# TurakhiaLab/TWILIGHT

Hardware: AMD Instinct MI355X
Metric: DP band cells/s, TALCO-XDrop progressive profile-profile alignment (bit-exact vs reference CPU path) (higher is better)
Workload: dtype f32

## Files before the change

### __graft_entry__.py

```python
from __future__ import annotations

import os
import subprocess
import sys

ROOT = os.path.dirname(os.path.abspath(__file__))
CSRC = os.path.join(ROOT, "twilight_amd", "csrc")
LIB = os.path.join(ROOT, "twilight_amd", "libtwl_align.so")
HIPCC = os.environ.get("HIPCC", "/opt/rocm/bin/hipcc")
KERNEL_SOURCES = ("twl_align.hip", "twl_knobs.inc.hip", "twl_launch.inc.hip", "twl_policy.inc.hip", "twl_run.inc.hip", "twl_comm.inc.hip", "talco_exit.hip.h", "talco_kernel.hip.h", "talco_nuc.hip.h", "talco_lds.hip.h", "talco_div.hip.h", "talco_team.hip.h", "talco_mt.hip.h", "talco_global.hip.h", "twl_level_plan.inc.hip", "twl_store.inc.hip", "twl_level.inc.hip", "level_kernels.hip.h", "restore_kernels.hip.h", "twl_place.inc.hip", "place_kernels.hip.h",
                  "twl_merge.inc.hip", "twl_merge_plan.inc.hip", "merge_kernels.hip.h", "twl_path_source.inc.hip", "twl_place_plan.inc.hip",
                  "twl_subtree.inc.hip", "twl_subtree_plan.inc.hip", "subtree_kernels.hip.h",
                  "twl_guide.inc.hip", "twl_guide_plan.inc.hip", "guide_kernels.hip.h",
                  "twl_guide_set.inc.hip", "twl_guide_set_plan.inc.hip", "guide_stage_kernels.hip.h",
                  "twl_strand.inc.hip", "twl_strand_plan.inc.hip", "strand_kernels.hip.h",
                  "twl_retree.inc.hip", "twl_retree_plan.inc.hip", "retree_kernels.hip.h",
                  "twl_retree_set.inc.hip", "twl_retree_set_plan.inc.hip", "retree_stage_kernels.hip.h",
                  "twl_backbone.inc.hip", "twl_backbone_plan.inc.hip", "backbone_kernels.hip.h",
                  "twl_keep.inc.hip", "twl_keep_plan.inc.hip", "keep_kernels.hip.h")
HIP_FLAGS = ["--offload-arch=gfx950", "-O2", "-ffp-contract=off", "-fno-slp-vectorize", "-fPIC", "-shared", "-std=c++17"]
HOST_FLAGS = ["-O2", "-std=c++17", "-fopenmp", "-ffp-contract=off", "-Wall"]

_STATE: dict = {}


def _digest(files, extra=()) -> str:
    import hashlib
    h = hashlib.sha256()
    for f in files:
        h.update(os.path.basename(f).encode() + b"\0")
        h.update(open(f, "rb").read())
    for e in extra:
        h.update(str(e).encode() + b"\0")
    return h.hexdigest()[:16]


def _stamped(target, stamp) -> bool:
    if not os.path.exists(target):
        return False
    return (b"TWLSTAMP:" + stamp.encode() + b";") in open(target, "rb").read()


def source_hash() -> str:
    import hashlib
    h = hashlib.sha256()
    for f in KERNEL_SOURCES:
        h.update(open(os.path.join(CSRC, f), "rb").read())
    return h.hexdigest()[:12]


def build_state() -> dict:
    return dict(_STATE)


def build() -> None:
    srcs = [os.path.join(CSRC, f) for f in KERNEL_SOURCES] + \
           [os.path.join(ROOT, "include", h) for h in ("twl_align.h", "twl_level.h", "twl_place.h", "twl_merge.h", "twl_subtree.h", "twl_guide.h", "twl_strand.h", "twl_retree.h", "twl_retree_set.h", "twl_backbone.h", "twl_keep.h")]
    flags = HIP_FLAGS + (["-DTWL_DEV"] if os.environ.get("TWL_DEV_BUILD") else [])
    stamp = _digest(srcs, flags)
    if _stamped(LIB, stamp):
        _STATE["libtwl_align.so"] = "current"
    else:
        subprocess.check_call([HIPCC] + flags + [f'-DTWL_SOURCE_HASH="{source_hash()}"', f'-DTWL_BUILD_STAMP="{stamp}"', "-o", LIB,
                               os.path.join(CSRC, "twl_align.hip")], cwd=CSRC)
        _STATE["libtwl_align.so"] = "built"
    host = os.path.join(CSRC, "host")
    lib_srcs = [os.path.join(host, f) for f in ("phylo.cpp", "seqdb_io.cpp", "helpers.cpp", "progressive.cpp", "driver.cpp", "align_gpu.cpp", "align_resident.cpp", "align_owned.cpp", "capi.cpp", "place.cpp", "merge.cpp", "partition.cpp", "subtrees.cpp", "guide.cpp", "retree.cpp", "place_tree.cpp", "strand.cpp")]
    hdrs = [os.path.join(host, h) for h in ("twl_host.hpp", "align_gpu.hpp", "level_policy.hpp", "exchange_plan.hpp", "guide_upgma.hpp", "guide_stage.hpp", "strand_orient.hpp")] + \
           [os.path.join(ROOT, "include", h) for h in ("twl_msa.h", "twl_align.h", "twl_level.h", "twl_place.h", "twl_merge.h", "twl_subtree.h", "twl_guide.h", "twl_strand.h", "twl_retree.h", "twl_retree_set.h", "twl_backbone.h", "twl_keep.h")] + \
           [os.path.join(CSRC, "twl_retree_plan.inc.hip")]
    hostlib = os.path.join(ROOT, "twilight_amd", "libtwl_host.so")
    hstamp = _digest(lib_srcs + hdrs, HOST_FLAGS + [stamp])
    if _stamped(hostlib, hstamp):
        _STATE["libtwl_host.so"] = "current"
    else:
        subprocess.check_call(["g++"] + HOST_FLAGS + [f'-DTWL_BUILD_STAMP="{hstamp}"', "-fPIC", "-shared", "-o", hostlib] + lib_srcs +
                              [LIB, "-Wl,-rpath,$ORIGIN", "-lz"], cwd=host)
        _STATE["libtwl_host.so"] = "built"
    exe = os.path.join(ROOT, "twilight_amd", "twilight-mi355x")
    exe_flags = HOST_FLAGS + ["-DTWL_PLACE", "-DTWL_MERGE", "-DTWL_SUBTREE", "-DTWL_GUIDE"]
    estamp = _digest([os.path.join(host, "main.cpp")] + hdrs, exe_flags + [hstamp])
    if _stamped(exe, estamp):
        _STATE["twilight-mi355x"] = "current"
    else:
        subprocess.check_call(["g++"] + exe_flags + [f'-DTWL_BUILD_STAMP="{estamp}"', "-o", exe, os.path.join(host, "main.cpp"),
                               hostlib, LIB, "-Wl,-rpath,$ORIGIN", "-lz"], cwd=host)
        _STATE["twilight-mi355x"] = "built"
    subprocess.check_call(["make", "-C", os.path.join(ROOT, "oracle"), "all"], stdout=subprocess.DEVNULL)
    sys.path.insert(0, ROOT)
    import twilight_amd

    twilight_amd.load_library()
    check_not_stale()
# ... 43 lines not shown
```

### include/twl_align.h

```cpp
#ifndef TWL_ALIGN_H
#define TWL_ALIGN_H

#include <stdint.h>

#ifdef __cplusplus
extern "C" {
#endif

#define TWL_MAX_MATRIX 21
#define TWL_MAX_MARKER 1024

enum twl_status {
    TWL_OK = 0,
    TWL_ERR_NOT_INITIALIZED = -1,
    TWL_ERR_BAD_ARGUMENT = -2,
    TWL_ERR_HIP = -3,
    TWL_ERR_UNSUPPORTED = -4
};

typedef struct twl_params {
    int32_t P;
    float   matrix[TWL_MAX_MATRIX * TWL_MAX_MATRIX];
    float   gap_open;
    float   gap_extend;
    float   gap_boundary;
    float   gap_char;
    int32_t xdrop;
    int32_t flen;
    int32_t marker;
} twl_params;

typedef struct twl_stats {
    uint64_t band_cells;
    uint64_t nominal_cells;
    double   kernel_ms;
    double   pack_ms;
    double   total_ms;
    int32_t  n_launches;
    int32_t  n_relaunched;
    int32_t  window;
    int32_t  grid;
    int32_t  matrix_mode;
    int32_t  speculative;
    int32_t  mt_tiles_predicted;
    int32_t  mt_tiles_inline;
    int32_t  mt_scouts_failed;
    int32_t  reserved;
    char     kernel[160];
} twl_stats;

int  twl_init(const int *device_ids, int n_devices);
void twl_shutdown(void);
const char *twl_last_error(void);
const char *twl_version(void);

int twl_align_batch(const twl_params *p, int32_t n_pairs, int32_t seq_len,
                    const float *freq, const float *gap_open, const float *gap_extend,
                    const int32_t *len, const int32_t *num,
                    int8_t *aln_out, int32_t *aln_len_out, int16_t *err_out);

int twl_align_batch_device(int device, void *stream, const twl_params *p, int32_t n_pairs, int32_t seq_len,
                           const float *d_freq, const float *d_gap_open, const float *d_gap_extend,
                           const int32_t *d_len, const int32_t *d_num,
                           int8_t *d_aln_out, int32_t *d_aln_len_out, int16_t *d_err_out);

void *twl_host_alloc(uint64_t bytes);
void  twl_host_free(void *p);

int twl_copy_to_device(int device, void *dst_dev, const void *src, uint64_t bytes);
int twl_copy_from_device(int device, void *dst, const void *src_dev, uint64_t bytes);
int twl_copy_rows_from_device(int device, void *dst, uint64_t dst_pitch, const void *src_dev, uint64_t src_pitch, uint64_t width, uint64_t rows);

int twl_get_stats(int device, twl_stats *out);

int twl_get_pair_cells(int device, uint64_t *cells_out, int32_t n);

int twl_column_scores(const twl_params *p, int32_t seq_len, const float *freq, const int32_t *len, const int32_t *num, float *out);

int twl_dp_column_scores(const twl_params *p, int32_t seq_len, const float *freq, const float *gap_open, const float *gap_extend,
                         const int32_t *len, const int32_t *num, float *out);

#define TWL_MT_REC_WORDS 12
typedef struct twl_mt_dims {
    int32_t n_run, slots, sp_pitch, segcap;
    int32_t n_scout, n_tile, rounds;
    int32_t lead2, marg, anchors;
    int32_t thr, small_tiles, marker;
    int32_t reserved[3];
} twl_mt_dims;
int twl_mt_tables(int device, twl_mt_dims *dims, int32_t *order, int32_t *anchor, int32_t *spath, int32_t *chain, int32_t *rec, int8_t *seg, int32_t *front);

#define TWL_COMM_ID_BYTES 128
int twl_comm_unique_id(void *id128);
int twl_comm_init(int device, int rank, int world, const void *id128);
int twl_comm_all_gather(int device, const void *d_send, void *d_recv, int64_t bytes_per_rank);
int twl_comm_all_gather_host(int device, const void *send, void *recv, int64_t bytes_per_rank);
int twl_comm_destroy(int device);

enum twl_knob { TWL_KNOB_MT_PERTURB = 1, TWL_KNOB_MT_MAX_PAIRS = 2, TWL_KNOB_MT_MIN_MARKER = 3, TWL_KNOB_MT_LEAD = 4, TWL_KNOB_MT_MARGIN = 5,
                TWL_KNOB_MT_ROUNDS = 6, TWL_KNOB_MT_THR_JOBS = 7, TWL_KNOB_FAIL_ROW_ALLOCS = 8,
                TWL_KNOB_PROT_MODE = 9, TWL_KNOB_ASSUME_ONEHOT_QUERY = 10, TWL_KNOB_MT_TAIL_PCT = 11, TWL_KNOB_MT_WIDE = 12, TWL_KNOB_NO_SPEC = 13, TWL_KNOB_SCOUT_XDROP_PCT = 14, TWL_KNOB_THR_SMALL = 15, TWL_KNOB_FORCE_GLOBAL = 16, TWL_KNOB_LEAF_STEP = 17, TWL_KNOB_POISON_TB = 18, TWL_KNOB_MT_ANCHOR = 19, TWL_KNOB_MT_LEAD2 = 20, TWL_KNOB_PROT_CORRIDOR = 21, TWL_KNOB_TAIL_OVERLAP = 22 };
int twl_set_knob(int key, int value);
int twl_plan_describe(const twl_params *p, int32_t n_pairs, const int32_t *len, int32_t num_cu, int32_t qry_onehot, int32_t wide_streak, char *out, int32_t cap);

#ifdef __cplusplus
}
#endif
#endif
```

### include/twl_level.h

```cpp
#ifndef TWL_LEVEL_H
#define TWL_LEVEL_H

#include "twl_align.h"

#ifdef __cplusplus
extern "C" {
#endif

typedef struct twl_store twl_store;

typedef struct twl_side {
    int32_t n_members;
    int32_t member_off;
    int32_t len;
    int32_t num;
    float   weight;
    int32_t cache_id;
    int32_t store_id;
    int32_t reserved;
} twl_side;

int  twl_store_create(int device, char type, int32_t n_seqs, const char *const *seqs, const int32_t *lens, twl_store **out);
void twl_store_destroy(twl_store *s);
int  twl_store_read_rows(twl_store *s, char *const *rows_out, int32_t *lens_out);
int  twl_store_read_rows_of(twl_store *s, int32_t n_ids, const int32_t *ids, char *out, int32_t *lens_out);
int  twl_store_write_rows(twl_store *s, int32_t n_ids, const int32_t *ids, const char *in, const int32_t *lens);
int  twl_store_write_cache(twl_store *s, int32_t id, const float *data, int32_t len);
int  twl_store_rows_to_block(twl_store *s, int32_t n_ids, const int32_t *ids, void *dev_block, int32_t *lens_out);
int  twl_store_rows_from_block(twl_store *s, int32_t n_ids, const int32_t *ids, const int32_t *lens, const void *dev_block);
int  twl_store_exchange_buffers(twl_store *s, int64_t send_bytes, int64_t recv_bytes, void **send_dev, void **recv_dev);
int  twl_store_read_cache(twl_store *s, int32_t id, float *out, int32_t *len_out);
int  twl_store_drop_cache(twl_store *s, int32_t id);

int twl_level_prepare(twl_store *s, const twl_params *p, float gappy_threshold, int32_t n_pairs, const twl_side *sides,
                      const int32_t *members, const float *member_weight, int32_t seq_len, int32_t *len_out, uint8_t *colinfo_out);

int twl_level_read_colinfo(twl_store *s, int32_t pair, int32_t side, uint8_t *out);
int twl_level_read_colinfo_many(twl_store *s, int32_t n_sel, const int32_t *pairs, uint8_t *out);

int twl_level_align(twl_store *s, const twl_params *p, const uint8_t *run_mask, int8_t *aln_out, int32_t *aln_len_out, int16_t *err_out);
int twl_level_align_mixed(twl_store *s, const twl_params *p, const uint8_t *run_mask, const uint8_t *zero_gap, int8_t *aln_out, int32_t *aln_len_out, int16_t *err_out);

int twl_level_read_path(twl_store *s, int32_t pair, int8_t *out, int32_t len);
int twl_level_read_paths(twl_store *s, int32_t n_sel, const int32_t *pairs, const int32_t *lens, int8_t *out, int32_t out_stride);

int twl_level_restore(twl_store *s, const twl_params *p, int32_t n_sel, const int32_t *pairs, int32_t out_stride, int32_t *final_len_out);
int twl_level_exchange_buffers(twl_store *s, int64_t send_bytes, int64_t recv_bytes, void **send_dev, void **recv_dev);
int twl_level_paths_to_block(twl_store *s, int32_t n_sel, const int32_t *pairs, const int32_t *lens, const uint8_t *where, void *blk_dev, const int64_t *blk_off);
int twl_level_paths_from_block(twl_store *s, int32_t n_sel, const int32_t *pairs, const int32_t *lens, const void *blk_dev, const int64_t *blk_off);
int twl_level_write_final(twl_store *s, int32_t pair, const int8_t *path, int32_t len);
int twl_level_read_final(twl_store *s, int32_t pair, int8_t *out, int32_t len);

int twl_level_commit(twl_store *s, const int8_t *paths, const int32_t *path_len, int32_t path_stride);

int twl_level_commit_from_dp(twl_store *s, const int8_t *paths, const int32_t *path_len, int32_t path_stride, const uint8_t *from_dp);

int twl_level_read_columns(twl_store *s, int32_t pair, int32_t side, float *out, int32_t max_cols);

int twl_level_timing(twl_store *s, double *prepare_ms, double *commit_ms);

#ifdef __cplusplus
}
#endif
#endif
```

### twilight_amd/api.py

```python
from __future__ import annotations

import ctypes as C
import os

import numpy as np

_HERE = os.path.dirname(os.path.abspath(__file__))
LIB_PATH = os.environ.get("TWL_LIB") or os.path.join(_HERE, "libtwl_align.so")
TWL_MAX_MATRIX = 21

_lib = None


class TwlError(RuntimeError):
    pass


class TwlParams(C.Structure):
    _fields_ = [("P", C.c_int32), ("matrix", C.c_float * (TWL_MAX_MATRIX * TWL_MAX_MATRIX)), ("gap_open", C.c_float),
                ("gap_extend", C.c_float), ("gap_boundary", C.c_float), ("gap_char", C.c_float), ("xdrop", C.c_int32),
                ("flen", C.c_int32), ("marker", C.c_int32)]


class TwlStats(C.Structure):
# ... 45 lines not shown
        lib.twl_set_knob.restype = C.c_int
        lib.twl_mt_tables.restype = C.c_int
        _lib = lib
    return _lib


def _check(rc):
    if rc != 0:
        raise TwlError(f"libtwl_align error {rc}: {load_library().twl_last_error().decode()}")


def make_params(matrix, *, gap_open=-50.0, gap_extend=-5.0, gap_boundary=None, gap_char=None, xdrop=None, flen=4096,
                marker=1024) -> TwlParams:
    m = np.asarray(matrix, dtype=np.float32)
    n = m.shape[0]
    p = TwlParams()
    p.P = n + 1
    flat = np.zeros(TWL_MAX_MATRIX * TWL_MAX_MATRIX, dtype=np.float32)
    flat[: n * n] = m.reshape(-1)
    p.matrix[:] = flat.tolist()
    p.gap_open = gap_open
    p.gap_extend = gap_extend
    p.gap_boundary = gap_extend if gap_boundary is None else gap_boundary
    p.gap_char = gap_extend if gap_char is None else gap_char
    p.xdrop = int(1000 * -gap_extend) if xdrop is None else int(xdrop)
    p.flen = flen
    p.marker = marker
    return p


def init(device_ids=None):
    lib = load_library()
    if device_ids is None:
        _check(lib.twl_init(None, 0))
    else:
        arr = (C.c_int * len(device_ids))(*device_ids)
        _check(lib.twl_init(arr, len(device_ids)))


def shutdown():
    load_library().twl_shutdown()


def _ptr(a, ty):
    return a.ctypes.data_as(C.POINTER(ty))


def align_batch(params: TwlParams, batch):
    lib = load_library()
    n, sl = batch.n_pairs, batch.seq_len
    freq = np.ascontiguousarray(batch.freq, dtype=np.float32)
    go = np.ascontiguousarray(batch.gap_open, dtype=np.float32)
    ge = np.ascontiguousarray(batch.gap_extend, dtype=np.float32)
    ln = np.ascontiguousarray(batch.len, dtype=np.int32)
    nm = np.ascontiguousarray(batch.num, dtype=np.int32)
    aln = np.zeros((n, 2 * sl), dtype=np.int8)
    aln_len = np.zeros(n, dtype=np.int32)
    err = np.zeros(n, dtype=np.int16)
    _check(lib.twl_align_batch(C.byref(params), C.c_int32(n), C.c_int32(sl), _ptr(freq, C.c_float), _ptr(go, C.c_float),
                               _ptr(ge, C.c_float), _ptr(ln, C.c_int32), _ptr(nm, C.c_int32), _ptr(aln, C.c_int8),
                               _ptr(aln_len, C.c_int32), _ptr(err, C.c_int16)))
    return aln, aln_len, err


def align_batch_device(params: TwlParams, n_pairs, seq_len, d_freq, d_gop, d_gex, d_len, d_num, d_aln, d_aln_len, d_err,
                       device=0, stream=None):
    lib = load_library()
    vp = C.c_void_p
    _check(lib.twl_align_batch_device(C.c_int(device), vp(stream or 0), C.byref(params), C.c_int32(n_pairs), C.c_int32(seq_len),
                                      vp(d_freq), vp(d_gop), vp(d_gex), vp(d_len), vp(d_num), vp(d_aln), vp(d_aln_len),
                                      vp(d_err)))


KNOB_MT_PERTURB, KNOB_MT_MAX_PAIRS, KNOB_MT_MIN_MARKER, KNOB_MT_LEAD, KNOB_MT_MARGIN, KNOB_MT_ROUNDS, KNOB_MT_THR_JOBS, KNOB_FAIL_ROW_ALLOCS = 1, 2, 3, 4, 5, 6, 7, 8
KNOB_PROT_MODE, KNOB_ASSUME_ONEHOT_QUERY, KNOB_MT_TAIL_PCT, KNOB_MT_WIDE, KNOB_NO_SPEC, KNOB_SCOUT_XDROP_PCT = 9, 10, 11, 12, 13, 14
KNOB_THR_SMALL = 15
KNOB_FORCE_GLOBAL = 16
KNOB_LEAF_STEP = 17
KNOB_POISON_TB = 18
KNOB_MT_ANCHOR = 19
KNOB_PROT_CORRIDOR = 21
KNOB_MT_LEAD2 = 20
KNOB_TAIL_OVERLAP = 22
PROT_MODES = {"auto": 0, "dense": 1, "sparse": 2, "presim": 3, "r1": 4, "lean_sparse": 5, "lean_presim": 6}


def set_knob(key: int, value: int):
    _check(load_library().twl_set_knob(C.c_int(key), C.c_int(value)))


def copy_to_device(dst_dev: int, data: bytes, device=0):
    _check(load_library().twl_copy_to_device(C.c_int(device), C.c_void_p(dst_dev), data, C.c_uint64(len(data))))


def copy_from_device(src_dev: int, n_bytes: int, device=0) -> bytes:
    buf = C.create_string_buffer(max(1, n_bytes))
    _check(load_library().twl_copy_from_device(C.c_int(device), buf, C.c_void_p(src_dev), C.c_uint64(n_bytes)))
    return buf.raw[:n_bytes]


def copy_rows_from_device(src_dev: int, src_pitch: int, width: int, rows: int, device=0) -> bytes:
    buf = C.create_string_buffer(max(1, width * rows))
    _check(load_library().twl_copy_rows_from_device(C.c_int(device), buf, C.c_uint64(width), C.c_void_p(src_dev), C.c_uint64(src_pitch), C.c_uint64(width), C.c_uint64(rows)))
    return buf.raw[: width * rows]


def plan_describe(params, lens, num_cu=256, qry_onehot=False, wide_streak=0, small_state=0) -> str:
    wide_streak = int(wide_streak) + (100000 * (32 + int(small_state)) if small_state else 0)
    lens = np.ascontiguousarray(lens, dtype=np.int32)
    buf = C.create_string_buffer(256)
    _check(load_library().twl_plan_describe(C.byref(params), C.c_int32(lens.shape[0]), _ptr(lens, C.c_int32), C.c_int32(num_cu), C.c_int32(int(qry_onehot)), C.c_int32(wide_streak), buf, C.c_int32(256)))
    return buf.value.decode()


def version() -> str:
    return load_library().twl_version().decode()


def get_stats(device=0) -> TwlStats:
    st = TwlStats()
    _check(load_library().twl_get_stats(C.c_int(device), C.byref(st)))
    return st


def get_pair_cells(n, device=0):
    out = np.zeros(n, dtype=np.uint64)
    _check(load_library().twl_get_pair_cells(C.c_int(device), _ptr(out, C.c_uint64), C.c_int32(n)))
    return out


def column_scores(params: TwlParams, ref: np.ndarray, qry: np.ndarray, ref_num: int, qry_num: int) -> np.ndarray:
    ref = np.ascontiguousarray(ref, dtype=np.float32)
    qry = np.ascontiguousarray(qry, dtype=np.float32)
    R, Q, P = ref.shape[0], qry.shape[0], ref.shape[1]
    sl = max(R, Q)
    freq = np.zeros((2, sl, P), dtype=np.float32)
    freq[0, :R] = ref
    freq[1, :Q] = qry
    ln = np.array([R, Q], dtype=np.int32)
    nm = np.array([ref_num, qry_num], dtype=np.int32)
    out = np.zeros((Q, R), dtype=np.float32)
    _check(load_library().twl_column_scores(C.byref(params), C.c_int32(sl), _ptr(freq, C.c_float), _ptr(ln, C.c_int32), _ptr(nm, C.c_int32), _ptr(out, C.c_float)))
    return out


def dp_column_scores(params: TwlParams, batch, pair: int = 0) -> np.ndarray:
    sl = batch.seq_len
    freq = np.ascontiguousarray(batch.freq[pair], dtype=np.float32)
    gop = np.ascontiguousarray(batch.gap_open[pair], dtype=np.float32)
    gex = np.ascontiguousarray(batch.gap_extend[pair], dtype=np.float32)
    ln = np.ascontiguousarray(batch.len[pair], dtype=np.int32)
    nm = np.ascontiguousarray(batch.num[pair], dtype=np.int32)
    out = np.zeros((int(ln[1]), int(ln[0])), dtype=np.float32)
    _check(load_library().twl_dp_column_scores(C.byref(params), C.c_int32(sl), _ptr(freq, C.c_float), _ptr(gop, C.c_float), _ptr(gex, C.c_float),
                                               _ptr(ln, C.c_int32), _ptr(nm, C.c_int32), _ptr(out, C.c_float)))
    return out


def mt_tables(device=0) -> dict:
    lib = load_library()
    dm = TwlMtDims()
    _check(lib.twl_mt_tables(C.c_int(device), C.byref(dm), None, None, None, None, None, None, None))
    n, s = dm.n_run, dm.slots
    order = np.zeros(n, dtype=np.int32)
    anchor = np.zeros((n, s), dtype=np.int32) if dm.anchors else None
    spath = np.zeros((n, dm.sp_pitch), dtype=np.int32)
# ... 10 lines not shown
```

### twilight_amd/csrc/host/align_resident.cpp

```cpp
#include "align_gpu.hpp"

#include <cstring>
#include <omp.h>

#include <algorithm>
#include <cstdio>
#include <cstdlib>
#include <iostream>
#include <string>
#include <thread>

namespace msa {
namespace progressive {
namespace gpu {

namespace {

inline twl_store *firstStore(const RunCtx &ctx) { return ctx.stores.empty() ? nullptr : ctx.stores[0]; }

std::vector<RunCtx::Raw> g_alnStage;
RunCtx::Raw g_finalStage, g_infoStage;

void createStore(RunCtx &ctx, SequenceDB *db, Option *option)
{
    const int n = (int)db->sequences.size();
    std::vector<const char *> rows(n);
    std::vector<int32_t> lens(n);
    for (int i = 0; i < n; ++i) {
        auto *s = db->sequences[i];
        if (s->id != i) { std::cerr << "ERROR: sequence ids are not dense.\n"; exit(1); }
        rows[i] = s->alnStorage[s->storage];
        lens[i] = s->len;
    }
    ctx.storeDev = selectedDevices();
    if (option->testVirtualDevices > 0) ctx.storeDev.assign((size_t)option->testVirtualDevices, selectedDevices()[0]);
    ctx.stores.assign(ctx.storeDev.size(), nullptr);
    std::vector<std::thread> th;
    std::vector<std::pair<int, std::string>> res(ctx.storeDev.size(), {TWL_OK, ""});
    for (size_t d = 0; d < ctx.storeDev.size(); ++d)
        th.emplace_back([&, d] {
            const int rc = twl_store_create(ctx.storeDev[d], option->type, n, rows.data(), lens.data(), &ctx.stores[d]);
            if (rc != TWL_OK) res[d] = {rc, twl_last_error()};
        });
    for (auto &t : th) t.join();
    for (auto &r : res)
        if (r.first != TWL_OK) { std::cerr << "ERROR: twl_store_create failed (" << r.first << "): " << r.second << '\n'; exit(1); }
    if (ctx.onStoreCreated) {
        const std::function<void(twl_store *)> hook = std::move(ctx.onStoreCreated);
        ctx.onStoreCreated = nullptr;
        for (twl_store *st : ctx.stores) hook(st);
    }
}

template <class F>
void onAllStores(RunCtx &ctx, const char *what, F fn)
{
    const size_t nd = ctx.stores.size();
    std::vector<std::pair<int, std::string>> res(nd, {TWL_OK, ""});
    if (nd == 1) { const int rc = fn(0); if (rc != TWL_OK) res[0] = {rc, twl_last_error()}; }
    else {
        std::vector<std::thread> th;
        for (size_t d = 0; d < nd; ++d)
            th.emplace_back([&, d] { const int rc = fn((int)d); if (rc != TWL_OK) res[d] = {rc, twl_last_error()}; });
        for (auto &t : th) t.join();
    }
    for (auto &r : res)
        if (r.first != TWL_OK) { std::cerr << "ERROR: " << what << " failed (" << r.first << "): " << r.second << '\n'; exit(1); }
}

void materialise(Tree *T, SequenceDB *db, Option *option)
{
    RunCtx &ctx = ctxOf(db);
    if (!firstStore(ctx)) return;
    const double t0 = nowMs();
    const int n = (int)db->sequences.size();
    std::vector<int32_t> lens(n);
    int rc = twl_store_read_rows(firstStore(ctx), nullptr, lens.data());
    if (rc != TWL_OK) die("twl_store_read_rows", rc);
    std::vector<char *> rows(n);
    size_t total = 0;
    for (int i = 0; i < n; ++i) total += (size_t)lens[i];
    free(db->rowArena);
    db->rowArena = static_cast<char *>(malloc(2 * total + 1));
    if (!db->rowArena) { std::cerr << "ERROR: out of host memory for the final rows.\n"; exit(1); }
    size_t at = 0;
    for (int i = 0; i < n; ++i) {
        auto *s = db->sequences[i];
        if (!s->borrowed) { free(s->alnStorage[0]); free(s->alnStorage[1]); }
        s->borrowed = true;
        s->alnStorage[s->storage] = db->rowArena + at;
        s->alnStorage[!s->storage] = db->rowArena + total + at;
        s->memLen = lens[i];
        rows[i] = s->alnStorage[s->storage];
// ... 142 lines not shown
    const int n = lv.n;
    std::vector<int32_t> lens(2 * (size_t)n);
    std::vector<std::vector<int32_t>> lensOf(lv.nd);
    onAllStores(ctx, "twl_level_prepare", [&](int d) {
        lensOf[d].resize(2 * (size_t)n);
        return twl_level_prepare(ctx.stores[d], &lv.tp, lv.option->gappyVertical, n, lv.sides.data(), lv.members.data(), lv.weights.data(), lv.stride,
                                 d == 0 ? lens.data() : lensOf[d].data(), nullptr);
    });
    for (int d = 1; d < lv.nd; ++d)
        if (lensOf[d] != lens) { std::cerr << "ERROR: device replicas disagree on the prepared level.\n"; exit(1); }
    lv.needsHost.assign(n, 0);
    for (int i = 0; i < n; ++i) {
        PairShape &s = lv.ps[i];
        s.lens = {lens[2 * i], lens[2 * i + 1]};
        if (s.lens.first != s.refLen || s.lens.second != s.qryLen) { lv.needInfo.push_back(i); lv.needsHost[i] = 1; }
    }
}

void fetchColumnInfo(const Level &lv, const std::vector<int> &which, bool wholeBlock, std::vector<ColumnInfo> &cols)
{
    if (which.empty()) return;
    const size_t stride = (size_t)lv.stride;
    uint8_t *info = reinterpret_cast<uint8_t *>(g_infoStage.get(2 * (wholeBlock ? (size_t)lv.n : which.size()) * stride));
    const int rc = wholeBlock ? twl_level_read_colinfo(firstStore(lv.ctx), -1, 0, info)
                              : twl_level_read_colinfo_many(firstStore(lv.ctx), (int32_t)which.size(), which.data(), info);
    if (rc != TWL_OK) die(wholeBlock ? "twl_level_read_colinfo" : "twl_level_read_colinfo_many", rc);
#pragma omp parallel for schedule(dynamic, 4)
    for (int t = 0; t < (int)which.size(); ++t) {
        const int i = which[t];
        const size_t slot = wholeBlock ? (size_t)i : (size_t)t;
        runsAndConsensus(&info[2 * slot * stride], lv.ps[i].refLen, lv.removal, lv.letters, cols[i].gappy.first, cols[i].consensus.first);
        runsAndConsensus(&info[(2 * slot + 1) * stride], lv.ps[i].qryLen, lv.removal, lv.letters, cols[i].gappy.second, cols[i].consensus.second);
    }
}

void planDp(Level &lv, PairRows &rows)
{
    const int n = lv.n;
    lv.maskZero.assign(n, 0);
    lv.takesPart.assign(n, 0);
    std::vector<long long> cost(n, 0);
    for (int i = 0; i < n; ++i) {
        const PairShape &s = lv.ps[i];
        rows.paths[i] = trivialPath(s);
        cost[i] = (long long)s.lens.first + s.lens.second;
        if (!goesToDp(s)) continue;
        lv.takesPart[i] = 1;
        lv.maskZero[i] = zeroGapChar(lv.task, s) ? 1 : 0;
    }
    lv.owner = dealPairs(cost, lv.takesPart, lv.route.procs ? lv.ctx.shard.world : lv.nd);
    lv.meBase = lv.route.procs ? lv.ctx.shard.rank : 0;
}

void addStats(const Level &lv, int d, bool firstCall, ReplicaShare &mine)
{
    const bool ownDevice = lv.nd == 1 || lv.ctx.storeDev[d] != lv.ctx.storeDev[(d + 1) % lv.nd];
    const bool nominal = firstCall && d == 0;
    twl_stats st{};
    if ((!ownDevice && !nominal) || twl_get_stats(lv.ctx.storeDev[d], &st) != TWL_OK) return;
    if (ownDevice) { foldStats(mine.part, st); mine.part.kernel_ms += st.kernel_ms; mine.totMs += st.total_ms; }
    if (nominal) mine.nominalCells += st.nominal_cells;
}

int retryDeferredPair(const Level &lv, int d, const std::vector<uint8_t> &mask, int8_t *aln, std::vector<int32_t> &alnLen, std::vector<int16_t> &err, ReplicaShare &mine)
{
    if (lv.n != 1) { std::cerr << "ERROR: a deferred-pass (task 1) level must hold exactly one pair; this one has " << lv.n << ".\n"; return (int)TWL_ERR_UNSUPPORTED; }
    if (!mask[0]) return (int)TWL_OK;
    twl_params tr = lv.maskZero[0] ? lv.tz : lv.tp;
    const uint8_t one = 1;
    int rc = TWL_OK;
    retryUntilPassed(tr, err[0], std::min(lv.ps[0].lens.first, lv.ps[0].lens.second), [&](const twl_params &grown) {
        if (lv.option->printDetail) std::cout << "Retry pair No. " << 0 << "\txdrop " << grown.xdrop << " flen " << grown.flen << '\n';
        const double tRetry = nowMs();
        rc = twl_level_align(lv.ctx.stores[d], &grown, &one, aln, alnLen.data(), err.data());
        if (rc != TWL_OK) return (int16_t)0;
        mine.callMs += nowMs() - tRetry;
        addStats(lv, d, false, mine);
        return err[0];
    });
    return rc;
}

int sortResults(const Level &lv, int d, const std::vector<uint8_t> &mask, const int8_t *aln, const std::vector<int32_t> &alnLen, const std::vector<int16_t> &err,
                PairRows &rows, ReplicaShare &mine)
{
    const size_t pitch = (size_t)2 * lv.stride;
    std::vector<int32_t> restore, restoreLen;
    for (int i = 0; i < lv.n; ++i) {
        if (!mask[i]) continue;
        rows.errs[i] = err[i];
        const int32_t len = (err[i] == 0) ? alnLen[i] : 0;
        if (!lv.route.inPlace) rows.paths[i].assign(&aln[i * pitch], &aln[i * pitch] + len);
        else if (lv.needsHost[i]) {
            if (len > 0 && !deferredLowQuality(lv.task, lv.ps[i])) { restore.push_back(i); restoreLen.push_back(len); } else rows.paths[i].clear();
        }
        else if (len > 0) { rows.fromDp[i] = 1; rows.dpLen[i] = len; }
    }
    if (restore.empty()) return (int)TWL_OK;
    std::vector<int32_t> fin(restore.size(), -1);
    const int rc = twl_level_restore(lv.ctx.stores[d], &lv.tp, (int32_t)restore.size(), restore.data(), lv.pathStride, fin.data());
    if (rc != TWL_OK) return rc;
    for (size_t t = 0; t < restore.size(); ++t) {
        if (fin[t] > 0) { rows.fromDp[restore[t]] = 2; rows.dpLen[restore[t]] = fin[t]; }
        else { mine.handedBack.push_back(restore[t]); mine.handedBackLen.push_back(restoreLen[t]); }
    }
    return (int)TWL_OK;
}

int alignShare(const Level &lv, int d, PairRows &rows, ReplicaShare &mine)
{
    const int n = lv.n;
    std::vector<uint8_t> mask(n, 0);
    int cnt = 0, cntZero = 0;
    for (int i = 0; i < n; ++i) if (lv.takesPart[i] && lv.owner[i] == lv.meBase + d) { mask[i] = 1; ++cnt; cntZero += lv.maskZero[i]; }
    if (!cnt) return (int)TWL_OK;
    int8_t *aln = lv.route.inPlace ? nullptr : reinterpret_cast<int8_t *>(g_alnStage[d].get((size_t)n * 2 * lv.stride));
    std::vector<int32_t> alnLen(n);
    std::vector<int16_t> err(n);
    const double tCall = nowMs();
    const int rc = (cntZero == cnt) ? twl_level_align(lv.ctx.stores[d], &lv.tz, mask.data(), aln, alnLen.data(), err.data())
                                    : twl_level_align_mixed(lv.ctx.stores[d], &lv.tp, mask.data(), cntZero ? lv.maskZero.data() : nullptr, aln, alnLen.data(), err.data());
    if (rc != TWL_OK) return rc;
    mine.callMs += nowMs() - tCall;
    addStats(lv, d, true, mine);
    if (lv.task == 1) {
        const int rr = retryDeferredPair(lv, d, mask, aln, alnLen, err, mine);
        if (rr != TWL_OK) return rr;
    }
    return sortResults(lv, d, mask, aln, alnLen, err, rows, mine);
}

#ifdef TWL_DEV
void dumpSchedule(const Level &lv, const PairRows &rows)
{
    const char *dump = getenv("TWL_DUMP_SCHEDULE");
    FILE *f = dump ? fopen(dump, "a") : nullptr;
    if (!f) return;
    std::vector<uint64_t> pc(lv.n, 0);
    if (lv.nd == 1) (void)twl_get_pair_cells(lv.ctx.storeDev[0], pc.data(), lv.n);
    for (int i = 0; i < lv.n; ++i)
        fprintf(f, "%d %d %d %d %d %d %d %llu\n", (int)lv.ctx.levels.size(), i, lv.nodes[i].first->seqsIncluded.empty() ? -1 : lv.nodes[i].first->seqsIncluded[0],
                lv.nodes[i].second->seqsIncluded.empty() ? -1 : lv.nodes[i].second->seqsIncluded[0], lv.ps[i].lens.first, lv.ps[i].lens.second, (int)rows.errs[i], (unsigned long long)pc[i]);
    fclose(f);
}
#endif

void mergeShares(const std::vector<ReplicaShare> &shares, RunCtx &ctx, LevelRecord &rec)
{
    double callMs = 0, totMs = 0;
    for (const ReplicaShare &s : shares) {
        callMs = std::max(callMs, s.callMs); totMs = std::max(totMs, s.totMs);
        rec.kernel_ms = std::max(rec.kernel_ms, s.part.kernel_ms);
        rec.band_cells += s.part.band_cells;
        rec.relaunched += s.part.relaunched;
    }
    const LevelRecord &p0 = shares[0].part;
    rec.matrix_mode = p0.matrix_mode; rec.speculative = p0.speculative; memcpy(rec.kernel, p0.kernel, sizeof rec.kernel);
    rec.mt_predicted += p0.mt_predicted; rec.mt_inline += p0.mt_inline;
    ctx.totals.call_ms += callMs;
    ctx.totals.total_ms += totMs;
    ctx.totals.nominal_cells += shares[0].nominalCells;
}

void postCheck(const Level &lv, int i, int alnRef, int alnQry)
{
    const PairShape &s = lv.ps[i];
    if (alnRef != s.refLen) std::cout << "R: Post " << lv.nodes[i].first->identifier << "(" << alnRef << "/" << s.refLen << ")\n";
    if (alnQry != s.qryLen) std::cout << "Q: Post " << lv.nodes[i].second->identifier << "(" << alnQry << "/" << s.qryLen << ")\n";
}

void joinHandedBack(const Level &lv, const ReplicaShare &share, PairRows &rows)
{
    const std::vector<int32_t> &fetch = share.handedBack;
    if (fetch.empty()) return;
    if (!lv.route.inPlace) { std::cerr << "ERROR: pairs handed back to the host outside the in-place mode.\n"; exit(1); }
    std::vector<int32_t> sideLen(2 * (size_t)lv.n);
    for (int i = 0; i < lv.n; ++i) { sideLen[2 * i] = lv.ps[i].refLen; sideLen[2 * i + 1] = lv.ps[i].qryLen; }
    const AlignedLevel al{lv.n, sideLen.data(), nullptr, nullptr, nullptr, lv.stride, lv.pathStride};
    const std::vector<int32_t> fin = restoreHandedBack(firstStore(lv.ctx), lv.param, *lv.option, al, fetch, share.handedBackLen,
                                                       [&](int i, int alnRef, int alnQry) { postCheck(lv, i, alnRef, alnQry); });
    for (size_t t = 0; t < fetch.size(); ++t) {
        rows.fromDp[fetch[t]] = 2; rows.dpLen[fetch[t]] = fin[t];
        rows.paths[fetch[t]].clear();
    }
}

void exchange(const Level &lv, RunCtx &ctx, PairRows &rows, LevelRecord &rec)
{
    if (!lv.route.devX) { exchangePaths(ctx, lv.owner, lv.takesPart, 2 * lv.stride, rows.paths, rows.errs, rec); return; }
    std::vector<int32_t> bound(lv.n);
    for (int i = 0; i < lv.n; ++i) bound[i] = lv.ps[i].refLen + lv.ps[i].qryLen;
    exchangeFinalPaths(ctx, firstStore(ctx), ctx.storeDev[0], lv.tp, lv.owner, lv.takesPart, bound, lv.pathStride, rows.fromDp, rows.dpLen, rows.errs, rec);
}

std::vector<int> judgeFailures(const Level &lv, PairRows &rows)
{
    std::vector<int> fallbackPairs;
    for (int i = 0; i < lv.n; ++i) {
        if (!deferFailedPair(lv.task, rows.errs[i])) continue;
        rows.paths[i].clear();
        rows.fromDp[i] = 0;
        fallbackPairs.push_back(i);
    }
    return fallbackPairs;
}

int8_t *finalPathsOnHost(const Level &lv, PairRows &rows, std::vector<int32_t> &finalLen, std::vector<char> &deferred)
{
    const int n = lv.n, pathStride = lv.pathStride;
    int8_t *finalPaths = reinterpret_cast<int8_t *>(g_finalStage.get((size_t)n * pathStride));
    std::vector<int> onHost;
    for (int i = 0; i < n; ++i) {
// ... 229 lines not shown
```

### twilight_amd/csrc/restore_kernels.hip.h

```cpp
#pragma once
#include "level_kernels.hip.h"

namespace twl {

constexpr int kNwCells = 4096;
constexpr int kNwRow = 128;

struct RestoreArgs {
    const int8_t *aln;
    const int32_t *aln_len;
    int32_t aln_stride;
    const uint8_t *colinfo;
    int32_t stride;
    const SideDesc *sides;
    const int32_t *len_red;
    const int32_t *sel;
    int32_t n_sel;
    int32_t *orig_idx;
    int32_t *run;
    int32_t *seg;
    int32_t *aoff;
    int32_t *both_list;
    int32_t *n_both;
    int32_t *wtot;
    int32_t n_wchunks;
    int8_t *arena;
    int32_t arena_stride;
    int32_t bstride;
    int8_t *out;
    int32_t out_stride;
    int32_t *out_len;
    int8_t *tbs;
    float *rows;
    float M[441];
    int32_t ms;
    float gap_open, gap_extend;
};

constexpr int kRsThreads = 1024, kRsItems = 16, kRsWaves = kRsThreads / 64;
constexpr int kRsItemsRuns = 8;

__global__ void __launch_bounds__(kRsThreads) restore_index_kernel(RestoreArgs a)
{
    __shared__ int s_wave[kRsWaves];
    const int side = 2 * a.sel[blockIdx.x >> 1] + (blockIdx.x & 1);
    const int len = a.sides[side].len;
    const uint8_t *ci = a.colinfo + (size_t)side * a.stride;
    int32_t *oi = a.orig_idx + (size_t)blockIdx.x * (size_t)(a.stride + 1);
    int base = 0;
    for (int c0 = 0; c0 < len; c0 += kRsThreads * kRsItems) {
        const int t0 = c0 + (int)threadIdx.x * kRsItems;
        bool keep[kRsItems];
        int cnt = 0;
#pragma unroll
        for (int k = 0; k < kRsItems; ++k) { const uint8_t f = ci[min(t0 + k, len - 1)]; keep[k] = (t0 + k < len) & !(f & 0x80); cnt += keep[k] ? 1 : 0; }
        int total;
        int dst = base + block_scan_int<kRsWaves>(cnt, &total, s_wave);
#pragma unroll
        for (int k = 0; k < kRsItems; ++k) if (keep[k]) oi[dst++] = t0 + k;
        base += total;
    }
    if (threadIdx.x == 0) oi[base] = len;
}

__global__ void __launch_bounds__(kRsThreads) restore_runs_kernel(RestoreArgs a)
{
    __shared__ int s_wave[kRsWaves];
    __shared__ int s_big;
    const int pair = a.sel[blockIdx.x];
    const int n = a.aln_len[pair];
    const int8_t *path = a.aln + (size_t)pair * a.aln_stride;
    const int32_t *oiR = a.orig_idx + (size_t)(2 * blockIdx.x) * (size_t)(a.stride + 1), *oiQ = oiR + (a.stride + 1);
    int32_t *runR = a.run + (size_t)blockIdx.x * 4 * a.bstride, *runQ = runR + a.bstride, *stR = runQ + a.bstride, *stQ = stR + a.bstride;
    int32_t *seg = a.seg + (size_t)blockIdx.x * a.bstride, *aoff = a.aoff + (size_t)blockIdx.x * a.bstride;
    int32_t *both_list = a.both_list + (size_t)blockIdx.x * a.bstride;
    if (threadIdx.x == 0) s_big = 0;
    int baseR = 0, baseQ = 0, baseA = 0, baseB = 0;
    bool tooBig = false;
    for (int c0 = 0; c0 <= n; c0 += kRsThreads * kRsItemsRuns) {
        const int b0 = c0 + (int)threadIdx.x * kRsItemsRuns;
        bool fR[kRsItemsRuns], fQ[kRsItemsRuns];
        int nR = 0, nQ = 0;
#pragma unroll
        for (int k = 0; k < kRsItemsRuns; ++k) {
            const int b = b0 + k;
            const int pv = path[max(min(b, n) - 1, 0)];
            const int prev = (b >= 1 && b <= n) ? pv : 3;
            fR[k] = (prev == 0) | (prev == 2); fQ[k] = (prev == 0) | (prev == 1);
            nR += fR[k] ? 1 : 0; nQ += fQ[k] ? 1 : 0;
        }
        int totR, totQ, totA, totB;
        int cR = baseR + block_scan_int<kRsWaves>(nR, &totR, s_wave);
        int cQ = baseQ + block_scan_int<kRsWaves>(nQ, &totQ, s_wave);
        int rR[kRsItemsRuns], rQ[kRsItemsRuns], sR[kRsItemsRuns], sQ[kRsItemsRuns];
        int sumA = 0, nB = 0;
#pragma unroll
        for (int k = 0; k < kRsItemsRuns; ++k) {
            const int b = b0 + k;
            cR += fR[k] ? 1 : 0; cQ += fQ[k] ? 1 : 0;
            const int iR = min(cR, a.stride), iQ = min(cQ, a.stride);
            const int pR = oiR[max(iR - 1, 0)], qR = oiR[iR], pQ = oiQ[max(iQ - 1, 0)], qQ = oiQ[iQ];
            const bool useR = (b <= n) & ((b == 0) | fR[k]), useQ = (b <= n) & ((b == 0) | fQ[k]);
            sR[k] = useR ? (cR ? pR + 1 : 0) : 0; rR[k] = useR ? qR - sR[k] : 0;
            sQ[k] = useQ ? (cQ ? pQ + 1 : 0) : 0; rQ[k] = useQ ? qQ - sQ[k] : 0;
            const bool both = rR[k] > 0 && rQ[k] > 0;
            if (both && ((long long)(rR[k] + 1) * (rQ[k] + 1) > kNwCells || rQ[k] + 1 > kNwRow)) tooBig = true;
            sumA += both ? rR[k] + rQ[k] : 0;
            nB += both ? 1 : 0;
        }
        int off = baseA + block_scan_int<kRsWaves>(sumA, &totA, s_wave);
        int lst = baseB + block_scan_int<kRsWaves>(nB, &totB, s_wave);
#pragma unroll
        for (int k = 0; k < kRsItemsRuns; ++k) {
            const int b = b0 + k;
            if (b > n) continue;
            const bool both = rR[k] > 0 && rQ[k] > 0;
            runR[b] = rR[k]; runQ[b] = rQ[k]; stR[b] = sR[k]; stQ[b] = sQ[k];
            seg[b] = both ? -1 : rR[k] + rQ[k];
            aoff[b] = off;
            if (both) { both_list[lst++] = b; off += rR[k] + rQ[k]; }
        }
        baseR += totR; baseQ += totQ; baseA += totA; baseB += totB;
    }
    __syncthreads();
    if (tooBig) s_big = 1;
    __syncthreads();
    if (threadIdx.x == 0) { a.out_len[pair] = s_big ? -1 : 0; a.n_both[blockIdx.x] = baseB; }
}

constexpr int kNwSmall = 31;
template <class L1, class L2, class Rows, class Tb>
__device__ __forceinline__ int nw_small(L1 s1, int m, L2 s2, int nn, const float *Mx, int ms, float go, float ge, Rows R, Tb T, int8_t *dst)
{
    const int W = nn + 1;
    int Mp = 0, Xp = 1, Yp = 2, Mc = 3, Xc = 4, Yc = 5;
    R(Mp, 0) = 0.0f; R(Xp, 0) = 0.0f; R(Yp, 0) = 0.0f; T(0) = 0;
    for (int j = 1; j <= nn; ++j) { R(Mp, j) = 0.0f; R(Yp, j) = 0.0f; R(Xp, j) = -1e9f; T(j) = 1; }
    for (int i = 1; i <= m; ++i) {
        const float *row = Mx + (size_t)(s1(i - 1) & 0x7f) * ms;
        R(Mc, 0) = 0.0f; R(Xc, 0) = 0.0f; R(Yc, 0) = -1e9f; T(i * W) = 2;
        float dM = R(Mp, 0), dX = R(Xp, 0), dY = R(Yp, 0), lM = 0.0f, lY = -1e9f;
        for (int j = 1; j <= nn; ++j) {
            const float base = row[s2(j - 1) & 0x7f];
            const float uM = R(Mp, j), uX = R(Xp, j), uY = R(Yp, j);
            const float mv = base + fmaxf(fmaxf(dM, dX), dY);
            const float xv = fmaxf(uM + go, uX + ge);
            const float yv = fmaxf(lM + go, lY + ge);
            const float best = fmaxf(fmaxf(mv, xv), yv);
            R(Mc, j) = mv; R(Xc, j) = xv; R(Yc, j) = yv;
            T(i * W + j) = (best == mv) ? 0 : ((best == yv) ? 1 : 2);
            dM = uM; dX = uX; dY = uY; lM = mv; lY = yv;
        }
        int t;
// ... 157 lines not shown
```

### twilight_amd/csrc/twl_align.hip

```cpp
#include "../../include/twl_align.h"
#include "../../include/twl_level.h"
#include "../../include/twl_place.h"
#include "../../include/twl_keep.h"
#include "../../include/twl_merge.h"
#include "../../include/twl_subtree.h"
#include "../../include/twl_guide.h"
#include "../../include/twl_strand.h"
#include "../../include/twl_retree.h"
#include "../../include/twl_retree_set.h"
#include "../../include/twl_backbone.h"
#include "level_kernels.hip.h"
#include "restore_kernels.hip.h"
#include "place_kernels.hip.h"
#include "keep_kernels.hip.h"
#include "merge_kernels.hip.h"
#include "subtree_kernels.hip.h"
#include "guide_kernels.hip.h"
#include "retree_kernels.hip.h"
#include "retree_stage_kernels.hip.h"
#include "backbone_kernels.hip.h"
#include "talco_kernel.hip.h"
#include "talco_nuc.hip.h"
#include "talco_global.hip.h"

#include <hip/hip_runtime.h>
#include <dlfcn.h>

#include <algorithm>
#include <atomic>
#include <chrono>
#include <cmath>
#include <cstdio>
#include <cstring>
#include <memory>
#include <mutex>
#include <numeric>
#include <string>
#include <thread>
#include <unordered_map>
#include <vector>

namespace twl {
struct FillJob { void *p; unsigned long long bytes; unsigned int val; };
struct FillArgs { FillJob j[8]; int n; };
__global__ void __launch_bounds__(256) fill_kernel(FillArgs a)
{
    const size_t t = (size_t)blockIdx.x * 256 + threadIdx.x, nt = (size_t)gridDim.x * 256;
    for (int r = 0; r < a.n; ++r) {
        const size_t nw = a.j[r].bytes >> 4;
        uint4 *w = reinterpret_cast<uint4 *>(a.j[r].p);
        const unsigned v = a.j[r].val;
        for (size_t i = t; i < nw; i += nt) w[i] = make_uint4(v, v, v, v);
        const size_t tail = a.j[r].bytes & 15;
        if (t < tail) reinterpret_cast<unsigned char *>(a.j[r].p)[(nw << 4) + t] = (unsigned char)v;
    }
}
__global__ void __launch_bounds__(256) collect_kernel(int n, const int16_t *err, const int32_t *aln_len, const unsigned long long *cells,
                                                      const unsigned long long *mt_stat, unsigned long long *out)
{
    const int i = blockIdx.x * 256 + threadIdx.x;
    unsigned long long *oc = out + 4;
    int32_t *ol = reinterpret_cast<int32_t *>(oc + n);
    int16_t *oe = reinterpret_cast<int16_t *>(ol + n);
    if (i < 4) out[i] = mt_stat ? mt_stat[i] : 0ull;
    if (i < n) { oc[i] = cells[i]; ol[i] = aln_len[i]; oe[i] = err[i]; }
    __threadfence_system();
}
}

namespace {

thread_local std::string g_err;
std::mutex g_mu;

static bool dbg_on() { static const bool v = getenv("TWL_DEBUG") != nullptr; return v; }
#define TRACE(...) do { if (dbg_on()) { fprintf(stderr, "[twl trace] " __VA_ARGS__); fputc('\n', stderr); fflush(stderr); } } while (0)

#define HIP_TRY(expr)                                                                                          \
    do {                                                                                                       \
        hipError_t e_ = (expr);                                                                                \
        if (e_ != hipSuccess) {                                                                                \
            g_err = std::string(#expr) + ": " + hipGetErrorString(e_);                                         \
            return TWL_ERR_HIP;                                                                                \
        }                                                                                                      \
    } while (0)


#include "twl_policy.inc.hip"

struct Buf {
    void *p = nullptr;
    size_t cap = 0;
    int ensure(size_t bytes)
    {
        if (bytes <= cap) return TWL_OK;
        if (p) (void)hipFree(p);
        p = nullptr; cap = 0;
        size_t want = bytes + bytes / 8 + 256;
        HIP_TRY(hipMalloc(&p, want));
        cap = want;
        return TWL_OK;
    }
    void release() { if (p) (void)hipFree(p); p = nullptr; cap = 0; }
};

struct Device {
    int id = 0;
    hipStream_t stream = nullptr;
    hipStream_t stream2 = nullptr;
    hipEvent_t ev2[2] = {};
    hipStream_t tail_stream = nullptr;
    hipEvent_t tail_ev[2] = {};
    Buf tb_tail;
    bool tail_side = false;
    bool fork_next = false;
    hipEvent_t ev[8] = {};
    int num_cu = 0;
    Buf cols, tb, cells, queue, items, errs, dbg;
    Buf gtb;
    Buf sim, sim_off, blk_off, m24;
    Buf team;
    Buf mt_chain, mt_rec, mt_seg, mt_spath, mt_stat, mt_jobs, mt_anchor;
    Buf simdump;
    bool dump_on = false;
    std::vector<int32_t> dbg_host;
    std::vector<int32_t> mt_jobs_host;
    twl_mt_dims mt_dims{};
    std::vector<int32_t> mt_order;
    bool mt_seen = false;
    Buf gc_zero;
    std::vector<uint8_t> gc_zero_host;
    std::vector<int16_t> last_err;
    void *probe_h = nullptr; size_t probe_cap = 0;
    PassMemory mem;
    int live_stores = 0;
    void *comm = nullptr;
    int comm_world = 0, comm_rank = 0;
    Buf comm_send, comm_recv;
    int mt_launch = 0;
    char kname[160] = {0};
    Buf h2d_freq, h2d_gop, h2d_gex, h2d_len, h2d_num, d_aln, d_alnlen, d_err;
    twl_stats stats{};
    std::vector<uint64_t> pair_cells;
    twl::FillArgs fills{};
    char *res_h = nullptr; size_t res_cap = 0;
    std::vector<int32_t> last_alnlen;
    std::mutex mu;
};

std::vector<Device *> g_devs;
bool g_init = false;

int find_dev(int device, Device **out)
{
    for (auto *d : g_devs) if (d->id == device) { *out = d; return TWL_OK; }
    g_err = "device not selected in twl_init";
    return TWL_ERR_BAD_ARGUMENT;
}

int flush_fills(Device *d, hipStream_t st)
{
    if (d->fills.n == 0) return TWL_OK;
    unsigned long long most = 0;
    for (int r = 0; r < d->fills.n; ++r) most = std::max(most, d->fills.j[r].bytes);
    const unsigned blocks = (unsigned)std::max<unsigned long long>(1, std::min<unsigned long long>((most / 16 + 255) / 256, (unsigned long long)d->num_cu * 8));
    hipLaunchKernelGGL(twl::fill_kernel, dim3(blocks), dim3(256), 0, st, d->fills);
    d->fills.n = 0;
    HIP_TRY(hipGetLastError());
    return TWL_OK;
}
int queue_fill(Device *d, hipStream_t st, void *p, size_t bytes, unsigned char v)
{
    if (!bytes) return TWL_OK;
    if (((size_t)p & 15) != 0) { HIP_TRY(hipMemsetAsync(p, v, bytes, st)); return TWL_OK; }
    if (d->fills.n == 8) { const int rc = flush_fills(d, st); if (rc) return rc; }
    d->fills.j[d->fills.n++] = twl::FillJob{p, (unsigned long long)bytes, 0x01010101u * v};
    return TWL_OK;
}
#define FILL_TRY(expr) do { const int rc_ = (expr); if (rc_) return rc_; } while (0)

int check_params(const twl_params *p)
{
    if (!p) { g_err = "params is null"; return TWL_ERR_BAD_ARGUMENT; }
    if (p->P != 6 && p->P != 22) { g_err = "profile width P must be 6 (nucleotide) or 22 (protein)"; return TWL_ERR_UNSUPPORTED; }
    if (p->marker < 2 || p->marker > TWL_MAX_MARKER) { g_err = "marker outside [2, TWL_MAX_MARKER]"; return TWL_ERR_UNSUPPORTED; }
    if (p->flen < 1) { g_err = "flen < 1"; return TWL_ERR_UNSUPPORTED; }
    if (p->xdrop < 0) { g_err = "xdrop < 0"; return TWL_ERR_BAD_ARGUMENT; }
    return TWL_OK;
}

#include "twl_knobs.inc.hip"
#include "twl_launch.inc.hip"
#include "twl_run.inc.hip"

}

static void twl_level_pool_release(Device *d);
namespace { extern int g_fail_next_row_allocs; void comm_destroy_raw(void *comm); }

extern "C" {

const char *twl_last_error(void) { return g_err.c_str(); }
#ifndef TWL_SOURCE_HASH
#define TWL_SOURCE_HASH "unstamped"
#endif
#ifndef TWL_BUILD_STAMP
#define TWL_BUILD_STAMP "unstamped"
#endif
__attribute__((used)) static const char twl_build_stamp[] = "TWLSTAMP:" TWL_BUILD_STAMP ";";
const char *twl_version(void) { return "twilight_amd 0.5 (gfx950) src " TWL_SOURCE_HASH; }

int twl_init(const int *device_ids, int n_devices)
{
    std::lock_guard<std::mutex> lk(g_mu);
    if (g_init) return TWL_OK;
    int count = 0;
    HIP_TRY(hipGetDeviceCount(&count));
    if (count < 1) { g_err = "no HIP device"; return TWL_ERR_HIP; }
    std::vector<int> ids;
    if (!device_ids || n_devices <= 0) ids.push_back(0);
    else ids.assign(device_ids, device_ids + n_devices);
    std::vector<Device *> devs;
    auto fail = [&](int rc) {
        for (auto *d : devs) {
            for (auto &e : d->ev) if (e) (void)hipEventDestroy(e);
            if (d->stream) (void)hipStreamDestroy(d->stream);
            if (d->stream2) (void)hipStreamDestroy(d->stream2);
            if (d->tail_stream) (void)hipStreamDestroy(d->tail_stream);
            for (auto &e : d->ev2) if (e) (void)hipEventDestroy(e);
// ... 48 lines not shown
                       &d->h2d_freq, &d->h2d_gop, &d->h2d_gex, &d->h2d_len, &d->h2d_num, &d->d_aln, &d->d_alnlen, &d->d_err})
            b->release();
        for (auto &e : d->ev) if (e) (void)hipEventDestroy(e);
        if (d->stream) (void)hipStreamDestroy(d->stream);
        if (d->stream2) (void)hipStreamDestroy(d->stream2);
        if (d->tail_stream) (void)hipStreamDestroy(d->tail_stream);
        for (auto &e : d->ev2) if (e) (void)hipEventDestroy(e);
        for (auto &e : d->tail_ev) if (e) (void)hipEventDestroy(e);
        if (d->res_h) (void)hipHostFree(d->res_h);
        if (d->probe_h) (void)hipHostFree(d->probe_h);
        delete d;
    }
    g_devs.clear();
    g_init = false;
}

int twl_align_batch_device(int device, void *stream, const twl_params *p, int32_t n_pairs, int32_t seq_len, const float *d_freq,
                           const float *d_gap_open, const float *d_gap_extend, const int32_t *d_len, const int32_t *d_num,
                           int8_t *d_aln_out, int32_t *d_aln_len_out, int16_t *d_err_out)
{
    if (!g_init) { g_err = "twl_init not called"; return TWL_ERR_NOT_INITIALIZED; }
    int rc = check_params(p);
    if (rc) return rc;
    if (n_pairs < 0 || seq_len < 1) { g_err = "bad n_pairs/seq_len"; return TWL_ERR_BAD_ARGUMENT; }
    Device *d = nullptr;
    if ((rc = find_dev(device, &d))) return rc;
    std::lock_guard<std::mutex> lk(d->mu);
    hipStream_t st = stream ? (hipStream_t)stream : d->stream;
    return run_device(d, st, p, n_pairs, seq_len, d_freq, d_gap_open, d_gap_extend, d_len, d_num, d_aln_out, d_aln_len_out,
                      d_err_out, nullptr);
}

static int run_host_slice(Device *d, const twl_params *p, const std::vector<int32_t> &ids, int32_t seq_len, const float *freq,
                          const float *gop, const float *gex, const int32_t *len, const int32_t *num, int8_t *aln_out,
                          int32_t *aln_len_out, int16_t *err_out)
{
    std::lock_guard<std::mutex> lk(d->mu);
    HIP_TRY(hipSetDevice(d->id));
    const int32_t n = (int32_t)ids.size();
    d->stats = twl_stats{};
    d->pair_cells.clear();
    if (n == 0) return TWL_OK;
    const size_t P = (size_t)p->P, sl = (size_t)seq_len;
    int rc;
    if ((rc = d->h2d_freq.ensure((size_t)n * 2 * sl * P * sizeof(float)))) return rc;
    if ((rc = d->h2d_gop.ensure((size_t)n * 2 * sl * sizeof(float)))) return rc;
    if ((rc = d->h2d_gex.ensure((size_t)n * 2 * sl * sizeof(float)))) return rc;
    if ((rc = d->h2d_len.ensure((size_t)n * 2 * sizeof(int32_t)))) return rc;
    if ((rc = d->h2d_num.ensure((size_t)n * 2 * sizeof(int32_t)))) return rc;
    if ((rc = d->d_aln.ensure((size_t)n * 2 * sl))) return rc;
    if ((rc = d->d_alnlen.ensure((size_t)n * sizeof(int32_t)))) return rc;
    if ((rc = d->d_err.ensure((size_t)n * sizeof(int16_t)))) return rc;
    hipStream_t st = d->stream;
    std::vector<int32_t> hl((size_t)n * 2), hn((size_t)n * 2);
    HIP_TRY(hipEventRecord(d->ev[5], st));
    bool contiguous = true;
    for (int32_t t = 0; t < n; ++t) contiguous = contiguous && ids[t] == ids[0] + t;
    for (int32_t t = 0; t < n; ++t) {
        const size_t s = (size_t)ids[t];
        hl[2 * t] = len[2 * s]; hl[2 * t + 1] = len[2 * s + 1];
        hn[2 * t] = num[2 * s]; hn[2 * t + 1] = num[2 * s + 1];
    }
    if (contiguous) {
        const size_t s0 = (size_t)ids[0];
        HIP_TRY(hipMemcpyAsync(d->h2d_freq.p, freq + s0 * 2 * sl * P, (size_t)n * 2 * sl * P * sizeof(float), hipMemcpyHostToDevice, st));
        HIP_TRY(hipMemcpyAsync(d->h2d_gop.p, gop + s0 * 2 * sl, (size_t)n * 2 * sl * sizeof(float), hipMemcpyHostToDevice, st));
        HIP_TRY(hipMemcpyAsync(d->h2d_gex.p, gex + s0 * 2 * sl, (size_t)n * 2 * sl * sizeof(float), hipMemcpyHostToDevice, st));
    } else {
        for (int32_t t = 0; t < n; ++t) {
            const size_t s = (size_t)ids[t];
            HIP_TRY(hipMemcpyAsync((float *)d->h2d_freq.p + (size_t)t * 2 * sl * P, freq + s * 2 * sl * P, 2 * sl * P * sizeof(float), hipMemcpyHostToDevice, st));
            HIP_TRY(hipMemcpyAsync((float *)d->h2d_gop.p + (size_t)t * 2 * sl, gop + s * 2 * sl, 2 * sl * sizeof(float), hipMemcpyHostToDevice, st));
            HIP_TRY(hipMemcpyAsync((float *)d->h2d_gex.p + (size_t)t * 2 * sl, gex + s * 2 * sl, 2 * sl * sizeof(float), hipMemcpyHostToDevice, st));
        }
    }
    HIP_TRY(hipMemcpyAsync(d->h2d_len.p, hl.data(), hl.size() * sizeof(int32_t), hipMemcpyHostToDevice, st));
    HIP_TRY(hipMemcpyAsync(d->h2d_num.p, hn.data(), hn.size() * sizeof(int32_t), hipMemcpyHostToDevice, st));
    rc = run_device(d, st, p, n, seq_len, (const float *)d->h2d_freq.p, (const float *)d->h2d_gop.p, (const float *)d->h2d_gex.p,
                    (const int32_t *)d->h2d_len.p, (const int32_t *)d->h2d_num.p, (int8_t *)d->d_aln.p, (int32_t *)d->d_alnlen.p,
                    (int16_t *)d->d_err.p, hl.data());
    if (rc) return rc;
    std::vector<int32_t> alen((size_t)n);
    std::vector<int16_t> aerr((size_t)n);
    HIP_TRY(hipMemcpyAsync(alen.data(), d->d_alnlen.p, alen.size() * sizeof(int32_t), hipMemcpyDeviceToHost, st));
    HIP_TRY(hipMemcpyAsync(aerr.data(), d->d_err.p, aerr.size() * sizeof(int16_t), hipMemcpyDeviceToHost, st));
    HIP_TRY(hipStreamSynchronize(st));
    size_t path_bytes = 0;
    for (int32_t t = 0; t < n; ++t) path_bytes += (size_t)std::max(alen[t], 0);
    const bool bulk = contiguous && path_bytes * 8 >= (size_t)n * 2 * sl;
    if (bulk) HIP_TRY(hipMemcpyAsync(aln_out + (size_t)ids[0] * 2 * sl, d->d_aln.p, (size_t)n * 2 * sl, hipMemcpyDeviceToHost, st));
    for (int32_t t = 0; t < n; ++t) {
        const size_t s = (size_t)ids[t];
        aln_len_out[s] = alen[t];
        err_out[s] = aerr[t];
        if (!bulk && alen[t] > 0)
            HIP_TRY(hipMemcpyAsync(aln_out + s * 2 * sl, (int8_t *)d->d_aln.p + (size_t)t * 2 * sl, (size_t)alen[t], hipMemcpyDeviceToHost, st));
    }
    HIP_TRY(hipEventRecord(d->ev[3], st));
    HIP_TRY(hipStreamSynchronize(st));
    float ms = 0.f;
    HIP_TRY(hipEventElapsedTime(&ms, d->ev[5], d->ev[3]));
    d->stats.total_ms = ms;
    return TWL_OK;
}

int twl_align_batch(const twl_params *p, int32_t n_pairs, int32_t seq_len, const float *freq, const float *gap_open,
                    const float *gap_extend, const int32_t *len, const int32_t *num, int8_t *aln_out, int32_t *aln_len_out,
                    int16_t *err_out)
{
    if (!g_init) { g_err = "twl_init not called"; return TWL_ERR_NOT_INITIALIZED; }
    int rc = check_params(p);
    if (rc) return rc;
    if (n_pairs < 0 || seq_len < 1 || (n_pairs > 0 && (!freq || !gap_open || !gap_extend || !len || !num || !aln_out || !aln_len_out || !err_out))) {
        g_err = "bad argument"; return TWL_ERR_BAD_ARGUMENT;
    }
    const size_t nd = g_devs.size();
    std::vector<int32_t> order((size_t)n_pairs);
    std::iota(order.begin(), order.end(), 0);
    std::stable_sort(order.begin(), order.end(), [&](int32_t x, int32_t y) {
        return (int64_t)len[2 * x] + len[2 * x + 1] > (int64_t)len[2 * y] + len[2 * y + 1];
    });
    std::vector<std::vector<int32_t>> slices(nd);
    if (nd == 1) { slices[0].resize((size_t)n_pairs); std::iota(slices[0].begin(), slices[0].end(), 0); }
    else for (size_t t = 0; t < order.size(); ++t) slices[t % nd].push_back(order[t]);
    if (nd == 1) return run_host_slice(g_devs[0], p, slices[0], seq_len, freq, gap_open, gap_extend, len, num, aln_out, aln_len_out, err_out);
    std::vector<int> rcs(nd, 0);
    std::vector<std::string> errs(nd);
    std::vector<std::thread> th;
    for (size_t i = 0; i < nd; ++i)
        th.emplace_back([&, i] {
            rcs[i] = run_host_slice(g_devs[i], p, slices[i], seq_len, freq, gap_open, gap_extend, len, num, aln_out, aln_len_out, err_out);
            errs[i] = g_err;
        });
    for (auto &t : th) t.join();
    for (size_t i = 0; i < nd; ++i) if (rcs[i]) { g_err = errs[i]; return rcs[i]; }
    return TWL_OK;
}

int twl_get_stats(int device, twl_stats *out)
{
    if (!g_init) { g_err = "twl_init not called"; return TWL_ERR_NOT_INITIALIZED; }
    if (!out) { g_err = "out is null"; return TWL_ERR_BAD_ARGUMENT; }
    Device *d = nullptr;
    int rc = find_dev(device, &d);
    if (rc) return rc;
    *out = d->stats;
    return TWL_OK;
}

int twl_column_scores(const twl_params *p, int32_t seq_len, const float *freq, const int32_t *len, const int32_t *num, float *out)
{
    if (!g_init) { g_err = "twl_init not called"; return TWL_ERR_NOT_INITIALIZED; }
    int rc = check_params(p);
    if (rc) return rc;
    if (seq_len < 1 || !freq || !len || !num || !out || len[0] < 1 || len[1] < 1 || len[0] > seq_len || len[1] > seq_len) { g_err = "bad argument"; return TWL_ERR_BAD_ARGUMENT; }
    Device *d = g_devs[0];
    std::lock_guard<std::mutex> lk(d->mu);
    HIP_TRY(hipSetDevice(d->id));
    hipStream_t st = d->stream;
    const size_t P = (size_t)p->P, sl = (size_t)seq_len, CW = P + 2;
    const int R = len[0], Q = len[1];
    const size_t pitch = ((size_t)Q + 63) & ~(size_t)63, simFloats = (size_t)(R + Q) * pitch;
    if ((rc = d->h2d_freq.ensure(2 * sl * P * sizeof(float)))) return rc;
    if ((rc = d->h2d_gop.ensure(2 * sl * sizeof(float)))) return rc;
    if ((rc = d->cols.ensure(2 * sl * CW * sizeof(float)))) return rc;
    if ((rc = d->h2d_len.ensure(2 * sizeof(int32_t)))) return rc;
    if ((rc = d->h2d_num.ensure(2 * sizeof(int32_t)))) return rc;
    if ((rc = d->items.ensure(sizeof(int32_t)))) return rc;
    if ((rc = d->sim.ensure(simFloats * sizeof(float)))) return rc;
// ... 66 lines not shown
    if (find_dev(device, &d)) return TWL_ERR_BAD_ARGUMENT;
    const size_t base = d->pair_cells.size() * 16 * sizeof(int32_t);
    if (!d->dbg.p || base + (size_t)n * 8 > d->dbg.cap) return TWL_ERR_BAD_ARGUMENT;
    return hipMemcpy(out, (const char *)d->dbg.p + base, (size_t)n * 8, hipMemcpyDeviceToHost) == hipSuccess ? TWL_OK : TWL_ERR_HIP;
}

void *twl_host_alloc(uint64_t bytes)
{
    void *p = nullptr;
    if (!g_init || bytes == 0) return nullptr;
    if (hipHostMalloc(&p, (size_t)bytes, hipHostMallocDefault) != hipSuccess) { (void)hipGetLastError(); return nullptr; }
    return p;
}

void twl_host_free(void *p)
{
    if (p) (void)hipHostFree(p);
}

int twl_copy_to_device(int device, void *dst_dev, const void *src, uint64_t bytes)
{
    if (!g_init) { g_err = "twl_init not called"; return TWL_ERR_NOT_INITIALIZED; }
    Device *d = nullptr;
    int rc = find_dev(device, &d);
    if (rc) return rc;
    if (bytes == 0) return TWL_OK;
    if (!dst_dev || !src) { g_err = "bad argument"; return TWL_ERR_BAD_ARGUMENT; }
    HIP_TRY(hipSetDevice(d->id));
    HIP_TRY(hipMemcpy(dst_dev, src, (size_t)bytes, hipMemcpyHostToDevice));
    return TWL_OK;
}

int twl_copy_from_device(int device, void *dst, const void *src_dev, uint64_t bytes)
{
    if (!g_init) { g_err = "twl_init not called"; return TWL_ERR_NOT_INITIALIZED; }
    Device *d = nullptr;
    int rc = find_dev(device, &d);
    if (rc) return rc;
    if (bytes == 0) return TWL_OK;
    if (!dst || !src_dev) { g_err = "bad argument"; return TWL_ERR_BAD_ARGUMENT; }
    HIP_TRY(hipSetDevice(d->id));
    HIP_TRY(hipMemcpy(dst, src_dev, (size_t)bytes, hipMemcpyDeviceToHost));
    return TWL_OK;
}

int twl_copy_rows_from_device(int device, void *dst, uint64_t dst_pitch, const void *src_dev, uint64_t src_pitch, uint64_t width, uint64_t rows)
{
    if (!g_init) { g_err = "twl_init not called"; return TWL_ERR_NOT_INITIALIZED; }
    Device *d = nullptr;
    int rc = find_dev(device, &d);
    if (rc) return rc;
    if (width == 0 || rows == 0) return TWL_OK;
    if (!dst || !src_dev || dst_pitch < width || src_pitch < width) { g_err = "bad argument"; return TWL_ERR_BAD_ARGUMENT; }
    HIP_TRY(hipSetDevice(d->id));
    HIP_TRY(hipMemcpy2D(dst, (size_t)dst_pitch, src_dev, (size_t)src_pitch, (size_t)width, (size_t)rows, hipMemcpyDeviceToHost));
    return TWL_OK;
}

int twl_set_knob(int key, int value)
{
    std::lock_guard<std::mutex> lk(g_mu);
    switch (key) {
    case TWL_KNOB_MT_PERTURB: g_mt_perturb = std::max(0, value); return TWL_OK;
    case TWL_KNOB_MT_MAX_PAIRS: g_mt_max_pairs = std::max(0, value); return TWL_OK;
    case TWL_KNOB_MT_MIN_MARKER: g_mt_min_marker = std::max(2, value); return TWL_OK;
    case TWL_KNOB_MT_LEAD: g_mt_lead = std::max(16, value); return TWL_OK;
    case TWL_KNOB_MT_MARGIN: if (value < 0) { g_mt_marg = 40; g_mt_marg_lat = 64; } else g_mt_marg = g_mt_marg_lat = std::max(2, value); return TWL_OK;
    case TWL_KNOB_MT_ROUNDS: g_mt_rounds = std::max(1, std::min(7, value)); return TWL_OK;
    case TWL_KNOB_MT_THR_JOBS: g_mt_thr_jobs = std::max(0, value); return TWL_OK;
    case TWL_KNOB_FAIL_ROW_ALLOCS: g_fail_next_row_allocs = std::max(0, value); return TWL_OK;
    case TWL_KNOB_PROT_MODE: if (value < 0 || value > 6) { g_err = "protein mode 0..6"; return TWL_ERR_BAD_ARGUMENT; } g_prot_mode = value; return TWL_OK;
    case TWL_KNOB_ASSUME_ONEHOT_QUERY: g_assume_onehot_query = value ? 1 : 0; return TWL_OK;
    case TWL_KNOB_MT_TAIL_PCT: g_mt_tail_pct = std::max(0, std::min(100, value)); return TWL_OK;
    case TWL_KNOB_MT_WIDE: g_mt_wide = value ? 1 : 0; return TWL_OK;
    case TWL_KNOB_NO_SPEC: g_no_spec = value ? 1 : 0; return TWL_OK;
    case TWL_KNOB_FORCE_GLOBAL: g_force_global = value ? 1 : 0; return TWL_OK;
    case TWL_KNOB_LEAF_STEP: g_leaf_step = value ? 1 : 0; return TWL_OK;
    case TWL_KNOB_POISON_TB: g_poison_tb = value ? 1 : 0; return TWL_OK;
    case TWL_KNOB_MT_ANCHOR: g_mt_anchor = value ? 1 : 0; return TWL_OK;
    case TWL_KNOB_MT_LEAD2: if (value < 0) { g_mt_lead2 = 96; g_mt_lead2_lat = 128; } else g_mt_lead2 = g_mt_lead2_lat = std::max(16, value); return TWL_OK;
    case TWL_KNOB_PROT_CORRIDOR: g_prot_corridor = std::max(0, value); for (auto *d : g_devs) d->mem.forget_corridor(); return TWL_OK;
    case TWL_KNOB_SCOUT_XDROP_PCT: g_scout_xdrop_pct = std::max(10, std::min(100, value)); return TWL_OK;
    case TWL_KNOB_TAIL_OVERLAP: g_tail_overlap = value ? 1 : 0; return TWL_OK;
    case TWL_KNOB_THR_SMALL: g_thr_small = std::max(0, std::min(2, value)); for (auto *d : g_devs) d->mem.forget_small(); return TWL_OK;
    default: g_err = "unknown knob"; return TWL_ERR_BAD_ARGUMENT;
    }
}

#include "twl_comm.inc.hip"

int twl_plan_describe(const twl_params *p, int32_t n_pairs, const int32_t *len, int32_t num_cu, int32_t qry_onehot, int32_t wide_streak, char *out, int32_t cap)
{
    if (!p || (p->P != 6 && p->P != 22) || n_pairs < 0 || (n_pairs > 0 && !len) || num_cu < 1 || !out || cap < 64) { g_err = "bad argument (nucleotide or protein parameters, a buffer of 64+ bytes)"; return TWL_ERR_BAD_ARGUMENT; }
    const PassMemory mem = memory_from_code(wide_streak);
    std::vector<int32_t> order;
    for (int32_t n = 0; n < n_pairs; ++n) if (len[2 * n] > 0 && len[2 * n + 1] > 0) order.push_back(n);
    std::stable_sort(order.begin(), order.end(), [&](int32_t x, int32_t y) { return (int64_t)len[2 * x] + len[2 * x + 1] > (int64_t)len[2 * y] + len[2 * y + 1]; });
    const int ms = p->P - 1;
    std::vector<float> M(p->matrix, p->matrix + ms * ms);
    if (p->P == 22) {
        ProtFacts pf;
        pf.n_run = (int)order.size(); pf.n_pairs = n_pairs; pf.num_cu = num_cu; pf.marker = p->marker; pf.M = M.data(); pf.gap_char = p->gap_char;
        pf.corridor_lost = mem.corridor_lost; pf.h_len = len; pf.order = order.data();
        const ProtPlan pl = plan_protein(pf, current_knobs());
        const int w = snprintf(out, (size_t)cap, "%s; mode %d; window %d", prot_first_name(pl.first), pl.mm, prot_first_window(pl.first));
        if (pl.presim && w > 0 && w < cap) snprintf(out + w, (size_t)(cap - w), "; %zu scores precomputed, corridor %d", pl.simFloats, pl.corridor);
        return TWL_OK;
    }
    NucFacts nf;
    nf.n_run = (int)order.size(); nf.num_cu = num_cu; nf.marker = p->marker; nf.M = M.data(); nf.gap_char = p->gap_char; nf.qry_onehot = qry_onehot != 0;
    nf.remember(mem); nf.h_len = len; nf.order = order.data();
    const NucPlan pl = plan_nucleotide(nf, current_knobs());
    snprintf(out, (size_t)cap, "%s; mode %d; window %d%s; bulk %d tail %d", nuc_first_name(pl.first), pl.mm5 ? 5 : pl.mm,
             pl.first == NucFirst::WideMt ? 3072 : ((pl.first == NucFirst::Throughput && pl.small) ? 512 : ((pl.first == NucFirst::Throughput && pl.four) ? 768 : 1024)), pl.probe ? " or 768 (a sample of the level decides)" : "", pl.bulk, pl.tail);
    return TWL_OK;
}

int twl_get_pair_cells(int device, uint64_t *cells_out, int32_t n)
{
    if (!g_init) { g_err = "twl_init not called"; return TWL_ERR_NOT_INITIALIZED; }
    Device *d = nullptr;
    int rc = find_dev(device, &d);
    if (rc) return rc;
    if (!cells_out || n < 0 || (size_t)n > d->pair_cells.size()) { g_err = "bad argument"; return TWL_ERR_BAD_ARGUMENT; }
    for (int32_t i = 0; i < n; ++i) cells_out[i] = d->pair_cells[i];
    return TWL_OK;
}

int twl_mt_tables(int device, twl_mt_dims *dims, int32_t *order, int32_t *anchor, int32_t *spath, int32_t *chain, int32_t *rec, int8_t *seg, int32_t *front)
{
    if (!g_init) { g_err = "twl_init not called"; return TWL_ERR_NOT_INITIALIZED; }
    Device *d = nullptr;
    int rc = find_dev(device, &d);
    if (rc) return rc;
    std::lock_guard<std::mutex> lk(d->mu);
    return read_mt_tables(d, dims, order, anchor, spath, chain, rec, seg, front);
}

}

#include "twl_level_plan.inc.hip"
#include "twl_store.inc.hip"
#include "twl_level.inc.hip"
#include "twl_place.inc.hip"
#include "twl_keep.inc.hip"
#include "twl_merge.inc.hip"
#include "twl_subtree.inc.hip"
#include "twl_guide.inc.hip"
#include "twl_guide_set.inc.hip"
#include "twl_strand.inc.hip"
#include "twl_retree.inc.hip"
#include "twl_retree_set.inc.hip"
#include "twl_backbone.inc.hip"
```

### twilight_amd/csrc/twl_knobs.inc.hip

```cpp

int g_prot_corridor = 448;
int g_mt_perturb = 0;
int g_mt_lead = 320, g_mt_marg = 40;
int g_mt_marg_lat = 64, g_mt_lead2_lat = 128;
int g_mt_anchor = 1, g_mt_lead2 = 96;
int g_mt_max_pairs = 1024, g_mt_min_marker = 512, g_mt_rounds = 2, g_mt_thr_jobs = 256;
int g_scout_xdrop_pct = 100;
int g_no_spec = 0;
int g_thr_small = 0;
int g_mt_wide = 1;
int g_mt_tail_pct = 70;
int g_prot_mode = 0;
int g_force_global = 0;
int g_assume_onehot_query = 0;
int g_leaf_step = 1;
int g_poison_tb = 0;
int g_tail_overlap = 1;
Knobs current_knobs()
{
    return Knobs{g_mt_max_pairs, g_mt_min_marker, g_mt_tail_pct, g_mt_wide, g_assume_onehot_query, g_no_spec, g_thr_small, (ProtMode)g_prot_mode, g_prot_corridor,
                 g_mt_thr_jobs, g_mt_rounds, g_mt_anchor, g_mt_lead, g_mt_marg, g_mt_marg_lat, g_mt_lead2, g_mt_lead2_lat};
}
```

### twilight_amd/csrc/twl_level.inc.hip

```cpp

namespace {

static_assert(sizeof(SideRow) == sizeof(twl::SideDesc) && offsetof(SideRow, weight) == offsetof(twl::SideDesc, weight) &&
              offsetof(SideRow, cache_slot) == offsetof(twl::SideDesc, cache_slot) && offsetof(SideRow, store_slot) == offsetof(twl::SideDesc, store_slot),
              "SideRow (twl_level_plan.inc.hip) is uploaded as twl::SideDesc");


int register_stored(twl_store *s, const PreparePlan &pp)
{
    std::vector<CacheEntry> fresh(pp.newIds.size());
    for (size_t k = 0; k < fresh.size(); ++k) {
        const int rc = fresh[k].take(s->d, pp.newLens[k], std::max<size_t>((size_t)pp.newLens[k] * (size_t)s->P * sizeof(float), 16));
        if (rc) return rc;
    }
    for (size_t k = 0; k < fresh.size(); ++k) s->cache[pp.newIds[k]] = std::move(fresh[k]);
    return TWL_OK;
}

int upload_prepare(twl_store *s, hipStream_t st, const PreparePlan &pp, const float *member_weight)
{
    LevelBufs *lv = s->lv;
    std::vector<float *> tab(pp.slotIds.size());
    for (size_t k = 0; k < tab.size(); ++k) tab[k] = (float *)s->cache.find(pp.slotIds[k])->second.buf.p;
    const size_t ns = pp.dsides.size();
// ... 85 lines not shown
}

int size_align(LevelBufs *lv, size_t n, size_t sl)
{
    int rc;
    if ((rc = lv->d_aln.ensure(n * 2 * sl))) return rc;
    if ((rc = lv->d_alnlen.ensure(n * sizeof(int32_t)))) return rc;
    return lv->d_err.ensure(n * sizeof(int16_t));
}

int read_back_align(twl_store *s, Device *d, hipStream_t st, int8_t *aln_out, int32_t *aln_len_out, int16_t *err_out)
{
    const int32_t n = s->n_pairs;
    const size_t sl = (size_t)s->seq_len;
    LevelBufs *lv = s->lv;
    if ((int32_t)d->last_err.size() == n && (int32_t)d->last_alnlen.size() == n) {
        std::copy(d->last_err.begin(), d->last_err.end(), err_out);
        std::copy(d->last_alnlen.begin(), d->last_alnlen.end(), aln_len_out);
        if (!aln_out) { d->stats.total_ms = d->stats.kernel_ms; return TWL_OK; }
    } else {
        HIP_TRY(hipMemcpyAsync(aln_len_out, lv->d_alnlen.p, (size_t)n * sizeof(int32_t), hipMemcpyDeviceToHost, st));
        HIP_TRY(hipMemcpyAsync(err_out, lv->d_err.p, (size_t)n * sizeof(int16_t), hipMemcpyDeviceToHost, st));
        HIP_TRY(hipStreamSynchronize(st));
    }
    int32_t ran = 0;
    for (int32_t i = 0; i < n; ++i) ran += aln_len_out[i] > 0;
    if (!aln_out) {}
    else if (ran * 2 >= n) HIP_TRY(hipMemcpyAsync(aln_out, lv->d_aln.p, (size_t)n * 2 * sl, hipMemcpyDeviceToHost, st));
    else
        for (int32_t i = 0; i < n; ++i)
            if (aln_len_out[i] > 0)
                HIP_TRY(hipMemcpyAsync(aln_out + (size_t)i * 2 * sl, (int8_t *)lv->d_aln.p + (size_t)i * 2 * sl, (size_t)aln_len_out[i], hipMemcpyDeviceToHost, st));
    HIP_TRY(hipEventRecord(d->ev[3], st));
    HIP_TRY(hipStreamSynchronize(st));
    float ms = 0.f;
    HIP_TRY(hipEventElapsedTime(&ms, d->ev[5], d->ev[3]));
    d->stats.total_ms = ms;
    return TWL_OK;
}


int size_restore(LevelBufs *lv, size_t ns, size_t n, size_t sl, unsigned nWch, unsigned nb, bool &soft)
{
    const size_t bstride = 2 * sl + 1;
    const struct { Buf *b; size_t bytes; bool soft; } want[] = {
        {&lv->r_oidx, 2 * ns * (sl + 1) * sizeof(int32_t), true},
        {&lv->r_run, ns * 4 * bstride * sizeof(int32_t), true},
        {&lv->r_seg, ns * bstride * sizeof(int32_t), true},
        {&lv->r_aoff, ns * bstride * sizeof(int32_t), true},
        {&lv->r_blist, ns * bstride * sizeof(int32_t), true},
        {&lv->r_nboth, ns * sizeof(int32_t), false},
        {&lv->r_wtot, ns * nWch * sizeof(int32_t), true},
        {&lv->r_arena, ns * 2 * sl, true},
        {&lv->r_outlen, n * sizeof(int32_t), false},
        {&lv->r_tb, ns * nb * twl::kNwThreads * (size_t)twl::kNwCells, true},
        {&lv->r_rows, ns * nb * twl::kNwThreads * 6 * (size_t)twl::kNwRow * sizeof(float), true},
    };
    for (const auto &w : want)
        if (const int rc = w.b->ensure(w.bytes)) { soft = w.soft; return rc; }
    return TWL_OK;
}

twl::RestoreArgs restore_args(const twl_store *s, const twl_params *p, int32_t n_sel, int32_t out_stride, unsigned nWch)
{
    const LevelBufs *lv = s->lv;
    const size_t sl = (size_t)s->seq_len;
    twl::RestoreArgs a{};
    a.aln = (const int8_t *)lv->d_aln.p; a.aln_len = (const int32_t *)lv->d_alnlen.p; a.aln_stride = (int32_t)(2 * sl);
    a.colinfo = (const uint8_t *)lv->d_colinfo.p; a.stride = s->seq_len;
    a.sides = lv->d_sides.as<const twl::SideDesc>(); a.len_red = (const int32_t *)lv->d_len.p;
    a.sel = lv->r_sel.as<const int32_t>(); a.n_sel = n_sel;
    a.orig_idx = (int32_t *)lv->r_oidx.p; a.run = (int32_t *)lv->r_run.p; a.seg = (int32_t *)lv->r_seg.p; a.aoff = (int32_t *)lv->r_aoff.p;
    a.both_list = (int32_t *)lv->r_blist.p; a.n_both = (int32_t *)lv->r_nboth.p;
    a.wtot = (int32_t *)lv->r_wtot.p; a.n_wchunks = (int32_t)nWch;
    a.arena = (int8_t *)lv->r_arena.p; a.arena_stride = (int32_t)(2 * sl); a.bstride = (int32_t)(2 * sl + 1);
    a.out = (int8_t *)lv->d_paths.p; a.out_stride = out_stride; a.out_len = (int32_t *)lv->r_outlen.p;
    a.tbs = (int8_t *)lv->r_tb.p; a.rows = (float *)lv->r_rows.p;
    a.ms = p->P - 1;
    for (int t = 0; t < a.ms * a.ms; ++t) a.M[t] = p->matrix[t];
    a.gap_open = p->gap_open; a.gap_extend = p->gap_extend;
    return a;
}

int restore_batch(twl_store *s, const twl_params *p, int32_t n_sel, const int32_t *pairs, int32_t out_stride, int32_t *final_len_out)
{
    int rc;
    const int32_t n = s->n_pairs;
    hipStream_t st = s->d->stream;
    LevelBufs *lv = s->lv;
    const size_t bstride = 2 * (size_t)s->seq_len + 1;
    {
        Arena &A = lv->up_restore;
        if ((rc = A.begin((size_t)n_sel * sizeof(int32_t), 1))) return rc;
        A.put(lv->r_sel, pairs, (size_t)n_sel);
        if ((rc = A.flush(st))) return rc;
    }
    const unsigned nWch = (unsigned)((bstride + (size_t)twl::kRsThreads * twl::kWrItems - 1) / ((size_t)twl::kRsThreads * twl::kWrItems));
    const unsigned nb = (unsigned)std::max(1, std::min(128, 4096 / n_sel));
    bool soft = false;
    if ((rc = size_restore(lv, (size_t)n_sel, (size_t)n, (size_t)s->seq_len, nWch, nb, soft))) {
        if (!soft) return rc;
        (void)hipGetLastError();
        for (int32_t t = 0; t < n_sel; ++t) final_len_out[t] = -1;
        return TWL_OK;
    }
    const twl::RestoreArgs a = restore_args(s, p, n_sel, out_stride, nWch);
    hipLaunchKernelGGL(twl::restore_index_kernel, dim3(2 * (unsigned)n_sel), dim3(twl::kRsThreads), 0, st, a);
    hipLaunchKernelGGL(twl::restore_runs_kernel, dim3((unsigned)n_sel), dim3(twl::kRsThreads), 0, st, a);
    hipLaunchKernelGGL(twl::restore_align_kernel, dim3((unsigned)n_sel, nb), dim3(twl::kNwThreads), 0, st, a);
    hipLaunchKernelGGL(twl::restore_count_kernel, dim3((unsigned)n_sel, nWch), dim3(twl::kRsThreads), 0, st, a);
    hipLaunchKernelGGL(twl::restore_write_kernel, dim3((unsigned)n_sel, nWch), dim3(twl::kRsThreads), 0, st, a);
    HIP_TRY(hipGetLastError());
    if ((rc = lv->back.ensure((size_t)n * sizeof(int32_t)))) return rc;
    HIP_TRY(hipMemcpyAsync(lv->back.p, lv->r_outlen.p, (size_t)n * sizeof(int32_t), hipMemcpyDeviceToHost, st));
    HIP_TRY(hipStreamSynchronize(st));
    const int32_t *all = (const int32_t *)lv->back.p;
    for (int32_t t = 0; t < n_sel; ++t) final_len_out[t] = all[pairs[t]];
    return TWL_OK;
}


int take_merged(twl_store *s, const int32_t *path_len, std::vector<CacheEntry> &merged)
{
    const CommitPlan &cp = s->commit;
    merged.resize(cp.nMerge());
    for (size_t k = 0; k < merged.size(); ++k) {
        const int32_t len = path_len[cp.merge[4 * k]];
        const int rc = merged[k].take(s->d, len, (size_t)len * (size_t)s->P * sizeof(float));
        if (rc) return rc;
    }
    return TWL_OK;
}

int stage_paths(twl_store *s, hipStream_t st, const int8_t *paths, const int32_t *path_len, int32_t path_stride, const uint8_t *from_dp)
{
    const size_t n = (size_t)s->n_pairs, ps = (size_t)path_stride;
    int rc;
    if ((rc = s->lv->d_paths.ensure(n * ps))) return rc;
    if (!from_dp) HIP_TRY(hipMemcpyAsync(s->lv->d_paths.p, paths, n * ps, hipMemcpyHostToDevice, st));
    else
        for (size_t i = 0; i < n; ++i)
            if (!from_dp[i] && path_len[i] > 0)
                HIP_TRY(hipMemcpyAsync((int8_t *)s->lv->d_paths.p + i * ps, paths + i * ps, (size_t)path_len[i], hipMemcpyHostToDevice, st));
    return s->lv->d_chunk.ensure(n * (size_t)s->commit.nChunks * 2 * sizeof(int32_t));
}

int upload_commit(twl_store *s, hipStream_t st, const std::vector<CacheEntry> &merged, const int32_t *path_len, const uint8_t *from_dp)
{
    const CommitPlan &cp = s->commit;
    LevelBufs *lv = s->lv;
    const size_t n = (size_t)s->n_pairs;
    std::vector<float *> &tab = s->h_tab;
    tab.clear();
    for (size_t k = 0; k < merged.size(); ++k)
        for (float *p : {(float *)s->cache.find(cp.mergeIds[2 * k])->second.buf.p, (float *)s->cache.find(cp.mergeIds[2 * k + 1])->second.buf.p, (float *)merged[k].buf.p})
            tab.push_back(p);
    Arena &A = lv->up_commit;
    int rc = A.begin((n + cp.work.size() + cp.merge.size()) * sizeof(int32_t) + cp.mergew.size() * sizeof(float) + tab.size() * sizeof(float *) + cp.mplane.size() + (from_dp ? n : 0), 7);
    if (rc) return rc;
    A.put(lv->d_pathlen, path_len, n);
    A.put(lv->d_work, cp.work);
    A.put(lv->d_merge, cp.merge);
    A.put(lv->d_mergew, cp.mergew);
    A.put(lv->d_tab, tab);
    A.put(lv->d_mplane, cp.mplane);
    if (from_dp) A.put(lv->d_fromdp, from_dp, n);
    return A.flush(st);
}

twl::CommitArgs commit_args(const twl_store *s, int32_t path_stride, bool fromDp)
{
    const LevelBufs *lv = s->lv;
    twl::CommitArgs a{};
    a.paths = (const int8_t *)lv->d_paths.p;
    if (fromDp) { a.from_dp = lv->d_fromdp.as<const uint8_t>(); a.paths_dp = (const int8_t *)lv->d_aln.p; a.dp_stride = (int32_t)(2 * (size_t)s->seq_len); }
    a.path_len = lv->d_pathlen.as<const int32_t>();
    a.path_stride = path_stride;
    a.chunk_base = (int32_t *)lv->d_chunk.p;
    a.n_chunks = s->commit.nChunks;
    a.sides = lv->d_sides.as<const twl::SideDesc>();
    a.member_seq = lv->d_mseq.as<const int32_t>();
    a.member_plane = lv->d_mplane.as<const uint8_t>();
    a.rows0 = (char *)s->rows[0].p; a.rows1 = (char *)s->rows[1].p;
    a.cap = s->cap;
    a.work = lv->d_work.as<const int32_t>();
    a.cache = lv->d_tab.as<float *const>();
    a.merge = lv->d_merge.as<const int32_t>();
    a.merge_w = lv->d_mergew.as<const float>();
    return a;
}

int rewrite_rows(twl_store *s, Device *d, hipStream_t st, const twl::CommitArgs &a)
{
    const CommitPlan &cp = s->commit;
    const dim3 grid(cp.nWork(), (unsigned)((cp.nChunks + 3) / 4));
    s->commit_side = false;
    if (!cp.nWork()) return TWL_OK;
    if (!cp.side) {
        const int rc = wait_rows(s, st);
// ... 117 lines not shown
        HIP_TRY(hipMemcpy(out, s->lv->d_colinfo.p, (size_t)s->n_pairs * 2 * (size_t)s->seq_len, hipMemcpyDeviceToHost));
        return TWL_OK;
    }
    const size_t idx = (size_t)pair * 2 + (size_t)side;
    const size_t len = (size_t)std::max(0, s->sides[idx].len);
    if (len) HIP_TRY(hipMemcpy(out, (const uint8_t *)s->lv->d_colinfo.p + idx * (size_t)s->seq_len, len, hipMemcpyDeviceToHost));
    return TWL_OK;
}

int twl_level_align(twl_store *s, const twl_params *p, const uint8_t *run_mask, int8_t *aln_out, int32_t *aln_len_out, int16_t *err_out)
{
    return twl_level_align_mixed(s, p, run_mask, nullptr, aln_out, aln_len_out, err_out);
}

int twl_level_align_mixed(twl_store *s, const twl_params *p, const uint8_t *run_mask, const uint8_t *zero_gap, int8_t *aln_out, int32_t *aln_len_out, int16_t *err_out)
{
    if (!s || !s->prepared) { g_err = "twl_level_prepare has not been called"; return TWL_ERR_BAD_ARGUMENT; }
    int rc = check_params(p);
    if (rc) return rc;
    if (p->P != s->P) { g_err = "params.P does not match the store's sequence type"; return TWL_ERR_BAD_ARGUMENT; }
    const int32_t n = s->n_pairs;
    if (n == 0) return TWL_OK;
    if (!aln_len_out || !err_out) { g_err = "bad argument"; return TWL_ERR_BAD_ARGUMENT; }
    DEVICE_CALL(call, s->d);
    Device *d = call.d;
    hipStream_t st = call.st;
    LevelBufs *lv = s->lv;
    const AlignPlan ap = plan_align(n, s->h_len, s->sides.data(), run_mask, g_leaf_step);
    if ((rc = upload_align(lv, st, ap.lm))) return rc;
    if ((rc = size_align(lv, (size_t)n, (size_t)s->seq_len))) return rc;
    HIP_TRY(hipEventRecord(d->ev[5], st));
    rc = run_device(d, st, p, n, s->seq_len, nullptr, nullptr, nullptr, lv->d_lenmask.as<const int32_t>(), lv->d_num.as<const int32_t>(), (int8_t *)lv->d_aln.p,
                    (int32_t *)lv->d_alnlen.p, (int16_t *)lv->d_err.p, ap.lm.data(), (const float *)lv->d_cols.p, ap.qryOneHot, zero_gap, ap.shape);
    if (rc) return rc;
    return read_back_align(s, d, st, aln_out, aln_len_out, err_out);
}

int twl_level_read_path(twl_store *s, int32_t pair, int8_t *out, int32_t len)
{
    if (!s || !s->prepared || !out || pair < 0 || pair >= s->n_pairs || len < 0 || len > 2 * s->seq_len || !s->lv || !s->lv->d_aln.p) { g_err = "bad argument"; return TWL_ERR_BAD_ARGUMENT; }
    DEVICE_CALL(call, s->d);
    if (len) HIP_TRY(hipMemcpy(out, (const int8_t *)s->lv->d_aln.p + (size_t)pair * 2 * (size_t)s->seq_len, (size_t)len, hipMemcpyDeviceToHost));
    return TWL_OK;
}

int twl_level_read_colinfo_many(twl_store *s, int32_t n_sel, const int32_t *pairs, uint8_t *out)
{
    if (!s || !s->prepared || n_sel < 0 || (n_sel > 0 && (!pairs || !out || !s->lv))) { g_err = "bad argument"; return TWL_ERR_BAD_ARGUMENT; }
    DEVICE_CALL(call, s->d);
    const size_t sl = (size_t)s->seq_len;
    for (int32_t t = 0; t < n_sel; ++t) {
        if (pairs[t] < 0 || pairs[t] >= s->n_pairs) { g_err = "pair index out of range"; return TWL_ERR_BAD_ARGUMENT; }
        HIP_TRY(hipMemcpyAsync(out + (size_t)t * 2 * sl, (const uint8_t *)s->lv->d_colinfo.p + (size_t)pairs[t] * 2 * sl, 2 * sl, hipMemcpyDeviceToHost, call.st));
    }
    HIP_TRY(hipStreamSynchronize(call.st));
    return TWL_OK;
}

int twl_level_read_paths(twl_store *s, int32_t n_sel, const int32_t *pairs, const int32_t *lens, int8_t *out, int32_t out_stride)
{
    if (!s || !s->prepared || n_sel < 0 || (n_sel > 0 && (!pairs || !lens || !out || !s->lv || !s->lv->d_aln.p)) || out_stride < 0) { g_err = "bad argument"; return TWL_ERR_BAD_ARGUMENT; }
    DEVICE_CALL(call, s->d);
    const size_t sl = (size_t)s->seq_len;
    for (int32_t t = 0; t < n_sel; ++t) {
        if (pairs[t] < 0 || pairs[t] >= s->n_pairs || lens[t] < 0 || lens[t] > out_stride || (size_t)lens[t] > 2 * sl) { g_err = "bad selection"; return TWL_ERR_BAD_ARGUMENT; }
        if (lens[t]) HIP_TRY(hipMemcpyAsync(out + (size_t)t * (size_t)out_stride, (const int8_t *)s->lv->d_aln.p + (size_t)pairs[t] * 2 * sl, (size_t)lens[t], hipMemcpyDeviceToHost, call.st));
    }
    HIP_TRY(hipStreamSynchronize(call.st));
    return TWL_OK;
}

int twl_level_restore(twl_store *s, const twl_params *p, int32_t n_sel, const int32_t *pairs, int32_t out_stride, int32_t *final_len_out)
{
    if (!s || !s->prepared || !s->lv || (n_sel > 0 && !s->lv->d_aln.p)) { g_err = "twl_level_align has not been called"; return TWL_ERR_BAD_ARGUMENT; }
    int rc = check_params(p);
    if (rc) return rc;
    const int32_t n = s->n_pairs;
    if (n_sel < 0 || (n_sel > 0 && (!pairs || !final_len_out)) || out_stride < 1) { g_err = "bad argument"; return TWL_ERR_BAD_ARGUMENT; }
    for (int32_t t = 0; t < n_sel; ++t) if (pairs[t] < 0 || pairs[t] >= n) { g_err = "pair index out of range"; return TWL_ERR_BAD_ARGUMENT; }
    DEVICE_CALL(call, s->d);
    if (s->staged_stride && s->staged_stride != out_stride) { g_err = "twl_level_restore: one row pitch per level"; return TWL_ERR_BAD_ARGUMENT; }
    if ((rc = s->lv->d_paths.ensure((size_t)n * (size_t)out_stride))) return rc;
    s->staged_stride = out_stride;
    constexpr int32_t kBatch = 4096;
    for (int32_t at = 0; at < n_sel; at += kBatch)
        if ((rc = restore_batch(s, p, std::min(kBatch, n_sel - at), pairs + at, out_stride, final_len_out + at))) return rc;
    return TWL_OK;
}

int twl_level_exchange_buffers(twl_store *s, int64_t send_bytes, int64_t recv_bytes, void **send_dev, void **recv_dev)
{
    if (!s || !s->prepared || !s->lv || send_bytes < 0 || recv_bytes < 0 || !send_dev || !recv_dev) { g_err = "bad argument"; return TWL_ERR_BAD_ARGUMENT; }
    DEVICE_CALL(call, s->d);
    int rc;
    if ((rc = s->lv->x_send.ensure(std::max<size_t>((size_t)send_bytes, 64)))) return rc;
    if ((rc = s->lv->x_recv.ensure(std::max<size_t>((size_t)recv_bytes, 64)))) return rc;
    *send_dev = s->lv->x_send.p; *recv_dev = s->lv->x_recv.p;
    return TWL_OK;
}

int twl_level_paths_to_block(twl_store *s, int32_t n_sel, const int32_t *pairs, const int32_t *lens, const uint8_t *where, void *blk_dev, const int64_t *blk_off)
{
    return level_rows_block(s, true, n_sel, pairs, lens, where, blk_dev, blk_off);
}

int twl_level_paths_from_block(twl_store *s, int32_t n_sel, const int32_t *pairs, const int32_t *lens, const void *blk_dev, const int64_t *blk_off)
{
    return level_rows_block(s, false, n_sel, pairs, lens, nullptr, const_cast<void *>(blk_dev), blk_off);
}

int twl_level_write_final(twl_store *s, int32_t pair, const int8_t *path, int32_t len)
{
    if (!s || !s->prepared || !s->lv || !s->staged_stride || pair < 0 || pair >= s->n_pairs || len < 0 || len > s->staged_stride || (len > 0 && !path)) { g_err = "bad argument (twl_level_restore first)"; return TWL_ERR_BAD_ARGUMENT; }
    DEVICE_CALL(call, s->d);
    if (len) HIP_TRY(hipMemcpy((int8_t *)s->lv->d_paths.p + (size_t)pair * (size_t)s->staged_stride, path, (size_t)len, hipMemcpyHostToDevice));
    return TWL_OK;
}

int twl_level_read_final(twl_store *s, int32_t pair, int8_t *out, int32_t len)
{
    if (!s || !s->prepared || !out || pair < 0 || pair >= s->n_pairs || len < 0 || !s->lv || !s->staged_stride || len > s->staged_stride) { g_err = "bad argument (twl_level_restore first)"; return TWL_ERR_BAD_ARGUMENT; }
    DEVICE_CALL(call, s->d);
    if (len) HIP_TRY(hipMemcpy(out, (const int8_t *)s->lv->d_paths.p + (size_t)pair * (size_t)s->staged_stride, (size_t)len, hipMemcpyDeviceToHost));
    return TWL_OK;
}

int twl_level_commit(twl_store *s, const int8_t *paths, const int32_t *path_len, int32_t path_stride)
{
    return twl_level_commit_from_dp(s, paths, path_len, path_stride, nullptr);
}

int twl_level_commit_from_dp(twl_store *s, const int8_t *paths, const int32_t *path_len, int32_t path_stride, const uint8_t *from_dp)
{
    if (!s || !s->prepared) { g_err = "twl_level_prepare has not been called"; return TWL_ERR_BAD_ARGUMENT; }
    const int32_t n = s->n_pairs;
    if (const char *why = check_commit(n, s->seq_len, s->staged_stride, s->lv && s->lv->d_aln.p, paths != nullptr, path_len, path_stride, from_dp)) { g_err = why; return TWL_ERR_BAD_ARGUMENT; }
    DEVICE_CALL(call, s->d);
    Device *d = call.d;
    hipStream_t st = call.st;
    s->prepared = false;
    s->staged_stride = 0;
    struct GiveBack { twl_store *s; ~GiveBack() { release_level(s->lv); } } giveBack{s};
    if (n == 0 || max_path(n, path_len) == 0) return TWL_OK;
    CommitPlan &cp = s->commit;
    plan_commit(cp, n, s->sides.data(), s->members, s->plane.data(), path_len, from_dp);
    int rc;
    if ((rc = grow_rows(s, cp.maxPath))) return rc;
    std::vector<CacheEntry> merged;
    if ((rc = take_merged(s, path_len, merged))) return rc;
    HIP_TRY(hipEventRecord(d->ev[6], st));
    if ((rc = stage_paths(s, st, paths, path_len, path_stride, from_dp))) return rc;
    if ((rc = upload_commit(s, st, merged, path_len, from_dp))) return rc;
    const twl::CommitArgs a = commit_args(s, path_stride, from_dp != nullptr);
    hipLaunchKernelGGL(twl::path_scan_kernel, dim3((unsigned)n), dim3(256), 0, st, a);
    if ((rc = rewrite_rows(s, d, st, a))) return rc;
    if (cp.nMerge()) {
        if (s->P == 6) hipLaunchKernelGGL(twl::merge_cache_kernel<6>, dim3(cp.nMerge(), (unsigned)cp.nChunks), dim3(256), 0, st, a);
        else hipLaunchKernelGGL(twl::merge_cache_kernel<22>, dim3(cp.nMerge(), (unsigned)cp.nChunks), dim3(256), 0, st, a);
    }
    HIP_TRY(hipGetLastError());
    HIP_TRY(hipEventRecord(d->ev[7], st));
    s->commit_pending = true;
    if (cp.hostRows) HIP_TRY(hipStreamSynchronize(st));
    apply_commit(s, merged);
    return TWL_OK;
}

int twl_level_read_columns(twl_store *s, int32_t pair, int32_t side, float *out, int32_t max_cols)
{
// ... 28 lines not shown
```

### twilight_amd/csrc/twl_run.inc.hip

```cpp

struct Call {
    Device *d; hipStream_t st; const twl_params *p;
    int32_t n_pairs, seq_len;
    const int32_t *d_len, *d_num; int32_t *d_alnlen; int16_t *d_err;
    const int32_t *h_len;
    std::vector<int32_t> len_host, order;
    int32_t n_run = 0;
    uint64_t nominal = 0;
    twl::KArgs a{};
    const int32_t *items() const { return (const int32_t *)d->items.p; }
    long long len_sum(int32_t pr) const { return (long long)h_len[2 * pr] + h_len[2 * pr + 1]; }
};
struct Results { std::vector<int16_t> err; std::vector<unsigned long long> cells; unsigned long long mt[4] = {0, 0, 0, 0}; };

int pinned_at_least(void **h, size_t *cap, size_t bytes)
{
    if (bytes <= *cap) return TWL_OK;
    if (*h) (void)hipHostFree(*h);
    *h = nullptr; *cap = 0;
    HIP_TRY(hipHostMalloc(h, bytes + bytes / 2, hipHostMallocDefault));
    *cap = bytes + bytes / 2;
    return TWL_OK;
}

// ... 165 lines not shown
    d->kname[0] = 0;
    return TWL_OK;
}

int first_throughput(Call &c, const NucPlan &pl, Ran &ran, int *grid, int *window)
{
    Device *d = c.d; hipStream_t st = c.st; const int32_t *items = c.items(); const int bulk = pl.bulk, tail = pl.tail;
    bool small = pl.small;
    int done = 0, rc;
    if (pl.probe && bulk >= 8 * d->num_cu && (rc = sample_small_window(c, pl, ran, grid, window, &small, &done))) return rc;
    const bool beside = tail > 0 && g_tail_overlap != 0;
    d->fork_next = beside;
    if (pl.four) rc = small ? launch_thr<4, 2, 5>(d, st, c.a, items + done, bulk - done, grid, window, pl.mm5, pl.sp)
                            : launch_thr<4, 3, 4>(d, st, c.a, items + done, bulk - done, grid, window, pl.mm5, pl.sp);
    else rc = with_mm<1, 0>(pl.mm, [&](auto MM) { return launch_lean<6, 8, 2, MM_OF(MM), 2>(d, st, c.a, items, bulk, grid, window); });
    ran.start = small ? Level::From512 : (pl.four ? Level::From768 : Level::Mid);
    const bool forked = beside && !d->fork_next;
    d->fork_next = false;
    if (rc || tail <= 0) return rc;
    const std::vector<int32_t> tailOrder(c.order.begin() + bulk, c.order.begin() + c.n_run);
    int g2 = 0, w2 = 0;
    ran.smallTiles = small && !ran.probed;
    ran.ranMt = true;
    hipStream_t ts = forked ? d->tail_stream : st;
    if (forked) HIP_TRY(hipStreamWaitEvent(d->tail_stream, d->tail_ev[0], 0));
    d->tail_side = forked;
    rc = with_mm<5, 2>(ran.mode, [&](auto MM) { return launch_mt<6, MM_OF(MM), 3, false, 4>(d, ts, c.a, items + bulk, tailOrder, tail, c.h_len, &g2, &w2, ran.smallTiles, pl.sp); });
    d->tail_side = false;
    if (!forked) return rc;
    if (!rc) rc = flush_fills(d, ts);
    else d->fills.n = 0;
    if (hipEventRecord(d->tail_ev[1], ts) != hipSuccess || hipStreamWaitEvent(st, d->tail_ev[1], 0) != hipSuccess) {
        (void)hipStreamSynchronize(ts);
        if (!rc) { g_err = "the join of a level's remainder with its bulk launch failed"; rc = TWL_ERR_HIP; }
    }
    return rc;
}

int first_nucleotide(Call &c, bool qry_onehot, int shape, Ran &ran, int *grid, int *window)
{
    Device *d = c.d; hipStream_t st = c.st; const twl::KArgs &a = c.a; const int32_t *items = c.items(); const int32_t n_run = c.n_run;
    NucFacts nf;
    nf.n_run = n_run; nf.num_cu = d->num_cu; nf.marker = c.p->marker; nf.M = a.M; nf.gap_char = c.p->gap_char; nf.qry_onehot = qry_onehot; nf.shape = shape; nf.dump = d->dump_on;
    nf.remember(d->mem); nf.h_len = c.h_len; nf.order = c.order.data();
    const NucPlan pl = plan_nucleotide(nf, current_knobs());
    if (pl.first == NucFirst::Throughput && (pl.small || pl.held_back)) d->mem.begin_small_level(n_run);
    const int mode = pl.mm5 ? 5 : pl.mm;
    ran.mode = mode;
    ran.leanMid = pl.lean && pl.mm == 2;
    ran.start = Level::Mid;
    TRACE("plan: %s%s, matrix mode %d%s", nuc_first_name(pl.first), pl.small ? " (512-row window, five workgroups per CU)" : "", pl.mm, pl.mm5 ? " (one-letter query rows)" : "");
    switch (pl.first) {
    case NucFirst::Dump:
        if (!pl.lean || n_run != 1) { g_err = "score dump: one pair, matrix within the fast-division range"; return TWL_ERR_UNSUPPORTED; }
        return with_mm<5, 2, 1, 0>(mode, [&](auto MM) { return launch_lean<6, 16, 1, MM_OF(MM), 1, false, true>(d, st, a, items, n_run, grid, window); });
    case NucFirst::WideMt:
        ran.spec = 3; ran.ranMt = true; ran.startedWide = true; ran.start = Level::Wide;
        return launch_mt<6, 2, 3, true, 4>(d, st, a, items, c.order, n_run, c.h_len, grid, window);
    case NucFirst::Mt:
        ran.smallTiles = nf.small_state > 0;
        ran.spec = 3; ran.ranMt = true;
        return launch_mt<6, 2, 3, false, 4>(d, st, a, items, c.order, n_run, c.h_len, grid, window, ran.smallTiles, pl.sp);
    case NucFirst::SpecShared:
        ran.mode = 2; ran.spec = 2;
        return launch_lean<6, 8, 2, 2, 4, true>(d, st, a, items, n_run, grid, window);
    case NucFirst::Spec16:
        ran.spec = 1;
        return with_mm<5, 2>(mode, [&](auto MM) { return launch_lean<6, 16, 1, MM_OF(MM), 1, true>(d, st, a, items, n_run, grid, window); });
    case NucFirst::Few16:
        return with_mm<5, 2, 1, 0>(mode, [&](auto MM) { return launch_lean<6, 16, 1, MM_OF(MM), 1>(d, st, a, items, n_run, grid, window); });
    case NucFirst::Throughput:
        return first_throughput(c, pl, ran, grid, window);
    default:
        return with_mm<2, 1, 0>(pl.mm, [&](auto MM) { return launch_dp<6, 8, 2, false, true, true, 4, MM_OF(MM)>(d, st, a, items, n_run, 0, grid, window); });
    }
}

int collect(Call &c, bool withMt, Results &res, bool withCells, unsigned long long *mt)
{
    Device *d = c.d; const int32_t n_pairs = c.n_pairs;
    hipLaunchKernelGGL(twl::collect_kernel, dim3((unsigned)((n_pairs + 255) / 256)), dim3(256), 0, c.st, (int)n_pairs, (const int16_t *)c.d_err, (const int32_t *)c.d_alnlen,
                       (const unsigned long long *)d->cells.p, withMt ? (const unsigned long long *)d->mt_stat.p : nullptr, (unsigned long long *)d->res_h);
    HIP_TRY(hipGetLastError());
    HIP_TRY(hipStreamSynchronize(c.st));
    const unsigned long long *r = (const unsigned long long *)d->res_h;
    const int32_t *rl = (const int32_t *)(r + 4 + n_pairs);
    const int16_t *re = (const int16_t *)(rl + n_pairs);
    std::copy(re, re + n_pairs, res.err.begin());
    d->last_alnlen.assign(rl, rl + n_pairs);
    if (withCells) std::copy(r + 4, r + 4 + n_pairs, res.cells.begin());
    if (mt) for (int t = 0; t < 4; ++t) mt[t] = r[t];
    return TWL_OK;
}

int launch_rung(Call &c, const Ran &ran, Rung rung, const std::vector<int32_t> &redo, int *g, int *w)
{
    Device *d = c.d; hipStream_t st = c.st; const twl::KArgs &a = c.a; const int32_t *it = c.items(); const int n = (int)redo.size();
    switch (rung) {
    case Rung::Guard:        return ran.prot ? launch_dp<22, 8, 2, false, true, true, 1, 3>(d, st, a, it, n, 0, g, w) : launch_dp<6, 16, 2, false, true, true, 1, 0>(d, st, a, it, n, 0, g, w);
    case Rung::Thr768:       return with_mm<5, 2>(ran.mode, [&](auto MM) { return launch_lean<6, 4, 3, MM_OF(MM), 4>(d, st, a, it, n, g, w); });
    case Rung::MtStitch1024: return with_mm<5, 2>(ran.mode, [&](auto MM) { return launch_mt<6, MM_OF(MM), 3, false, 4>(d, st, a, it, redo, n, c.h_len, g, w); });
    case Rung::Lean1024:     return with_mm<5, 2>(ran.mode, [&](auto MM) { return launch_lean<6, 8, 2, MM_OF(MM), 4>(d, st, a, it, n, g, w); });
    case Rung::Prot16:       return launch_lean<22, 16, 1, 3, 1>(d, st, a, it, n, g, w);
    case Rung::Mt3072:       return launch_mt<6, 2, 3, true, 4>(d, st, a, it, redo, n, c.h_len, g, w);
    case Rung::Lean2048:     return launch_lean<6, 8, 4, 2, 2>(d, st, a, it, n, g, w);
    case Rung::Ieee16x2:     return launch_dp<6, 16, 2, false, true, true, 1, 0>(d, st, a, it, n, 0, g, w);
    case Rung::Wide4608:     return ran.prot ? launch_dp<22, 8, 9, false, false, false>(d, st, a, it, n, 1, g, w) : launch_dp<6, 8, 9, false, false, true>(d, st, a, it, n, 1, g, w);
    default:                 return ran.prot ? launch_global<22>(d, st, a, it, n, c.seq_len, g, w) : launch_global<6>(d, st, a, it, n, c.seq_len, g, w);
    }
}
int timed_rerun(Call &c, const Ran &ran, Rung rung, const std::vector<int32_t> &redo, float *ms_redo, int *window)
{
    Device *d = c.d;
    HIP_TRY(hipMemcpyAsync(d->items.p, redo.data(), redo.size() * sizeof(int32_t), hipMemcpyHostToDevice, c.st));
    HIP_TRY(hipEventRecord(d->ev[3], c.st));
    int grid2 = 0;
    TRACE("re-run: %d pairs on %s", (int)redo.size(), rung_name(rung));
    FILL_TRY(launch_rung(c, ran, rung, redo, &grid2, window));
    HIP_TRY(hipEventRecord(d->ev[4], c.st));
    HIP_TRY(hipStreamSynchronize(c.st));
    float ms = 0.f;
    HIP_TRY(hipEventElapsedTime(&ms, d->ev[3], d->ev[4]));
    *ms_redo += ms;
    d->stats.n_launches += 1;
    d->stats.n_relaunched += (int32_t)redo.size();
    return TWL_OK;
}
std::vector<int32_t> pairs_with(const std::vector<int16_t> &err, int16_t code, int16_t code2)
{
    std::vector<int32_t> v;
    for (int32_t n = 0; n < (int32_t)err.size(); ++n) if (err[n] == code || err[n] == code2) v.push_back(n);
    return v;
}

int climb_ladder(Call &c, const Ran &ran, Results &res, LadderOutcome &o, float *ms_redo)
{
    const Knobs k = current_knobs();
    int rc, w2 = 0;
    if ((rc = collect(c, ran.ranMt, res, true, ran.ranMt ? res.mt : nullptr))) return rc;
    TRACE("dp kernel done");
    o.firstInline = res.mt[1];
    for (Level at = ran.start; at != Level::Global;) {
        std::vector<int32_t> redo = pairs_with(res.err, twl::kErrGuard, twl::kErrGuard);
        const RedoKind kind = redo.empty() ? RedoKind::Overflow : RedoKind::Guard;
        if (kind == RedoKind::Overflow) redo = pairs_with(res.err, twl::kErrOverflow, twl::kErrOverflow);
        if (redo.empty()) break;
        RedoFacts f;
        f.count = (int)redo.size(); f.marker = c.p->marker; f.dump = c.d->dump_on;
        for (int32_t n : redo) f.sumLen += c.len_sum(n);
        const Step s = next_rung(ran, at, kind, f, k);
        if (kind == RedoKind::Guard) o.guardRound = true;
        else if (at == Level::From512) o.from512Pairs = f.count;
        if (s.rung == Rung::Mt3072 || s.rung == Rung::Lean2048) o.widePairs += f.count;
        if (s.rung == Rung::Mt3072 || s.rung == Rung::MtStitch1024) o.redoMt = true;
        if ((rc = timed_rerun(c, ran, s.rung, redo, ms_redo, &w2))) return rc;
        o.relaunched += f.count;
        at = s.next;
        if (at != Level::Global && (rc = collect(c, ran.ranMt || o.redoMt, res, false, nullptr))) return rc;
    }
    if (o.relaunched > 0) {
        unsigned long long now[4];
        if ((rc = collect(c, ran.ranMt || o.redoMt, res, true, now))) return rc;
        if (o.redoMt) for (int t = 0; t < 4; ++t) res.mt[t] += now[t];
    }
    return TWL_OK;
}
// ... 91 lines not shown
```

### twilight_amd/csrc/twl_store.inc.hip

```cpp
#include <cstdlib>
#include "twl_path_source.inc.hip"

namespace {

struct DeviceCall {
    Device *d;
    hipStream_t st;
    std::lock_guard<std::mutex> lk;
    int rc;
    explicit DeviceCall(Device *dev) : d(dev), st(dev->stream), lk(dev->mu), rc(make_current()) {}
    int make_current() { HIP_TRY(hipSetDevice(d->id)); return TWL_OK; }
};
#define DEVICE_CALL(name, dev) DeviceCall name(dev); if (name.rc) return name.rc

}

struct Ref {
    void *p = nullptr;
    template <class T> T *as() const { return static_cast<T *>(p); }
};
struct PinBuf {
    void *p = nullptr;
    size_t cap = 0;
    int ensure(size_t bytes)
// ... 101 lines not shown
}
void release_level(LevelBufs *&lv) { if (lv) { lv->busy = false; lv = nullptr; } }

std::vector<Buf> &cache_pool(Device *d)
{
    static std::mutex mu;
    static std::unordered_map<Device *, std::vector<Buf>> pools;
    std::lock_guard<std::mutex> lk(mu);
    return pools[d];
}
int cache_buf_get(Device *d, Buf &b, size_t bytes)
{
    auto &pool = cache_pool(d);
    size_t best = pool.size();
    for (size_t k = 0; k < pool.size(); ++k)
        if (pool[k].cap >= bytes && (best == pool.size() || pool[k].cap < pool[best].cap)) best = k;
    if (best != pool.size()) { b = pool[best]; pool[best] = pool.back(); pool.pop_back(); return TWL_OK; }
    b = Buf{};
    return b.ensure(bytes + bytes / 4);
}
void cache_buf_put(Device *d, Buf &b)
{
    if (!b.p) return;
    auto &pool = cache_pool(d);
    if (pool.size() >= 4096) {
        size_t small = 0;
        for (size_t k = 1; k < pool.size(); ++k) if (pool[k].cap < pool[small].cap) small = k;
        if (pool[small].cap < b.cap) std::swap(pool[small], b);
        b.release();
        return;
    }
    pool.push_back(b);
    b = Buf{};
}

struct CacheEntry {
    Device *d = nullptr;
    Buf buf;
    int32_t len = 0;
    CacheEntry() = default;
    CacheEntry(CacheEntry &&o) noexcept : d(o.d), buf(o.buf), len(o.len) { o.buf = Buf{}; }
    CacheEntry &operator=(CacheEntry &&o) noexcept
    {
        if (this != &o) { cache_buf_put(d, buf); d = o.d; buf = o.buf; len = o.len; o.buf = Buf{}; }
        return *this;
    }
    ~CacheEntry() { cache_buf_put(d, buf); }
    int take(Device *dev, int32_t n, size_t bytes) { d = dev; len = n; return cache_buf_get(dev, buf, bytes); }
};
}

static void twl_level_pool_release(Device *d)
{
    auto &pool = level_pool(d);
    for (const auto &b : pool) b->release_all();
    pool.clear();
    for (Buf &b : cache_pool(d)) b.release();
    cache_pool(d).clear();
}

struct twl_store {
    Device *d = nullptr;
    int P = 6;
    char type = 'n';
    int32_t n_seqs = 0;
    int64_t cap = 0;
    Buf rows[2];
    std::vector<uint8_t> plane;
    std::vector<int32_t> len;
    std::unordered_map<int32_t, CacheEntry> cache;
    Buf lut;
    int32_t n_pairs = 0, seq_len = 0;
    bool prepared = false;
    std::vector<twl_side> sides;
    std::vector<int32_t> members;
    std::vector<int32_t> h_len, h_num;
    CommitPlan commit;
    std::vector<float *> h_tab;
    bool commit_pending = false;
    bool commit_side = false;
    hipEvent_t rows_event = nullptr;
    LevelBufs *lv = nullptr;
    int32_t staged_stride = 0;
    Arena up_rows;
    Buf d_gather;
    Buf x_send, x_recv;
    double prepare_ms = 0, commit_ms = 0;
    double squeeze_ms = 0;
};

namespace {

void build_lut(char type, uint8_t *lut)
{
    for (int c = 0; c < 256; ++c) {
        const int u = (c >= 'a' && c <= 'z') ? c - 32 : c;
        int v;
        if (type == 'n') {
            switch (u) {
            case 'A': v = 0; break;
            case 'C': v = 1; break;
            case 'G': v = 2; break;
            case 'T': case 'U': v = 3; break;
            case '-': case '.': v = 5; break;
            default: v = 4; break;
            }
        } else {
            static const char acids[] = "ACDEFGHIKLMNPQRSTVWY";
            v = 20;
            for (int k = 0; k < 20; ++k) if (u == acids[k]) v = k;
            if (u == '-' || u == '.') v = 21;
        }
        lut[c] = (uint8_t)v;
    }
}

int64_t rows_budget_cap(twl_store *s)
{
    size_t freeB = 0, totalB = 0;
    if (hipMemGetInfo(&freeB, &totalB) != hipSuccess) { (void)hipGetLastError(); return INT64_MAX; }
    const int64_t budget = (int64_t)(totalB / 6);
    return std::max<int64_t>(256, budget / (2 * std::max<int64_t>(1, s->n_seqs)));
}

int g_fail_next_row_allocs = 0;

int grow_rows(twl_store *s, int64_t need, int64_t want = 0)
{
    if (need <= s->cap) return TWL_OK;
    Device *d = s->d;
    HIP_TRY(hipStreamSynchronize(d->stream2));
    s->rows_event = nullptr;
    const int64_t minCap = (need + 255) & ~(int64_t)255;
    int64_t ncap = std::max(need, std::min(std::max(want, need + need / 2), rows_budget_cap(s)));
    ncap = (ncap + 255) & ~(int64_t)255;
    Buf nb[2];
    auto alloc_both = [&](int64_t cap) {
        for (int pl = 0; pl < 2; ++pl) {
            int rc = TWL_ERR_HIP;
            if (g_fail_next_row_allocs > 0) { --g_fail_next_row_allocs; g_err = "row allocation failed (test knob)"; }
            else rc = nb[pl].ensure((size_t)s->n_seqs * (size_t)cap);
            if (rc) { nb[0].release(); nb[1].release(); (void)hipGetLastError(); return rc; }
        }
        return (int)TWL_OK;
    };
    int rc = alloc_both(ncap);
    if (rc && ncap > minCap) { ncap = minCap; rc = alloc_both(ncap); }
    if (rc) return rc;
    for (int pl = 0; pl < 2; ++pl)
        if (s->rows[pl].p)
            HIP_TRY(hipMemcpy2DAsync(nb[pl].p, (size_t)ncap, s->rows[pl].p, (size_t)s->cap, (size_t)s->cap, (size_t)s->n_seqs, hipMemcpyDeviceToDevice, d->stream));
    HIP_TRY(hipStreamSynchronize(d->stream));
    for (int pl = 0; pl < 2; ++pl) { s->rows[pl].release(); s->rows[pl] = nb[pl]; }
    s->cap = ncap;
    return TWL_OK;
}

struct StoreEnd {
    void operator()(twl_store *raw) const
    {
        std::unique_ptr<twl_store> s(raw);
        (void)hipSetDevice(s->d->id);
        (void)hipStreamSynchronize(s->d->stream);
        (void)hipStreamSynchronize(s->d->stream2);
        s->cache.clear();
        release_level(s->lv);
// ... 286 lines not shown
```

### twilight_amd/level.py

```python
from __future__ import annotations

import ctypes as C
from dataclasses import dataclass
from typing import List, Optional, Sequence

import numpy as np

from . import api


class TwlSide(C.Structure):
    _fields_ = [("n_members", C.c_int32), ("member_off", C.c_int32), ("len", C.c_int32), ("num", C.c_int32), ("weight", C.c_float),
                ("cache_id", C.c_int32), ("store_id", C.c_int32), ("reserved", C.c_int32)]


_SYMBOLS = ["twl_store_create", "twl_store_destroy", "twl_store_read_rows", "twl_store_read_rows_of", "twl_store_write_rows", "twl_store_write_cache", "twl_store_rows_to_block", "twl_store_rows_from_block", "twl_store_exchange_buffers", "twl_store_read_cache", "twl_store_drop_cache",
            "twl_level_prepare", "twl_level_read_colinfo", "twl_level_read_colinfo_many", "twl_level_align", "twl_level_align_mixed", "twl_level_read_path", "twl_level_read_paths", "twl_level_commit", "twl_level_commit_from_dp", "twl_level_read_columns", "twl_level_timing",
            "twl_level_restore", "twl_level_read_final", "twl_level_exchange_buffers", "twl_level_paths_to_block", "twl_level_paths_from_block",
            "twl_level_write_final"]


def exported_symbols():
    return list(_SYMBOLS)


def _lib():
    lib = api.load_library()
    for name in _SYMBOLS:
        if name != "twl_store_destroy":
            getattr(lib, name).restype = C.c_int
    lib.twl_store_destroy.restype = None
    return lib


@dataclass
class Side:
    members: Sequence[int]
    member_weight: Sequence[float]
    len: int
    num: int
    weight: float
    cache_id: int = -1
    store_id: int = -1


class Store:

    def __init__(self, seqs: List[bytes], seq_type: str = "n", device: int = 0):
        lib = _lib()
        self.P = 6 if seq_type == "n" else 22
        self.n = len(seqs)
        arr = (C.c_char_p * self.n)(*seqs)
        lens = (C.c_int32 * self.n)(*[len(s) for s in seqs])
        self._h = C.c_void_p()
        api._check(lib.twl_store_create(C.c_int(device), C.c_char(seq_type.encode()), C.c_int32(self.n), arr, lens, C.byref(self._h)))
        self._n_pairs = 0
        self._seq_len = 0
        self._dependants = []

    def close(self):
        for d in list(getattr(self, "_dependants", ())):
            d.close()
        if self._h:
            _lib().twl_store_destroy(self._h)
            self._h = C.c_void_p()

    def __del__(self):
        try:
            self.close()
        except Exception:
            pass

    def rows(self) -> List[bytes]:
        lib = _lib()
        lens = (C.c_int32 * self.n)()
        api._check(lib.twl_store_read_rows(self._h, None, lens))
        bufs = [C.create_string_buffer(max(int(n), 1)) for n in lens]
        ptrs = (C.c_void_p * self.n)(*[C.cast(b, C.c_void_p) for b in bufs])
        api._check(lib.twl_store_read_rows(self._h, ptrs, lens))
        return [bufs[i].raw[: lens[i]] for i in range(self.n)]

    def rows_of(self, ids: Sequence[int]) -> List[bytes]:
        lib = _lib()
        n = len(ids)
        idv = (C.c_int32 * n)(*ids)
        lens = (C.c_int32 * n)()
        api._check(lib.twl_store_read_rows_of(self._h, C.c_int32(n), idv, None, lens))
        buf = C.create_string_buffer(max(1, sum(lens)))
        api._check(lib.twl_store_read_rows_of(self._h, C.c_int32(n), idv, buf, lens))
        out, at = [], 0
        for k in range(n):
            out.append(buf.raw[at: at + lens[k]])
            at += lens[k]
        return out

    def write_rows(self, ids: Sequence[int], rows: Sequence[bytes], via_device_block: bool = False):
        lib = _lib()
        n = len(ids)
        idv = (C.c_int32 * n)(*ids)
        lens = (C.c_int32 * n)(*[len(r) for r in rows])
        blob = b"".join(rows)
        if not via_device_block:
# ... 26 lines not shown
        prof = np.ascontiguousarray(profile, dtype=np.float32)
        api._check(_lib().twl_store_write_cache(self._h, C.c_int32(cache_id), prof.ctypes.data_as(C.POINTER(C.c_float)), C.c_int32(prof.shape[0])))

    def cache(self, cache_id: int) -> np.ndarray:
        lib = _lib()
        n = C.c_int32(0)
        api._check(lib.twl_store_read_cache(self._h, C.c_int32(cache_id), None, C.byref(n)))
        out = np.zeros((n.value, self.P), dtype=np.float32)
        api._check(lib.twl_store_read_cache(self._h, C.c_int32(cache_id), out.ctypes.data_as(C.POINTER(C.c_float)), C.byref(n)))
        return out

    def prepare(self, params: api.TwlParams, pairs: Sequence[Sequence[Side]], gappy_threshold: float = 0.95, seq_len: Optional[int] = None):
        lib = _lib()
        n = len(pairs)
        sides = (TwlSide * (2 * n))()
        members, weights = [], []
        for i, pr in enumerate(pairs):
            for sd in range(2):
                s = pr[sd]
                x = sides[2 * i + sd]
                x.n_members, x.member_off, x.len, x.num, x.weight = len(s.members), len(members), s.len, s.num, s.weight
                x.cache_id, x.store_id, x.reserved = s.cache_id, s.store_id, 0
                members.extend(int(m) for m in s.members)
                weights.extend(s.member_weight)
        sl = seq_len if seq_len is not None else max([1] + [s.len for pr in pairs for s in pr])
        mem = np.asarray(members, dtype=np.int32)
        w = np.asarray(weights, dtype=np.float32)
        lens = np.zeros((n, 2), dtype=np.int32)
        info = np.zeros((n, 2, sl), dtype=np.uint8)
        api._check(lib.twl_level_prepare(self._h, C.byref(params), C.c_float(gappy_threshold), C.c_int32(n), sides,
                                         mem.ctypes.data_as(C.POINTER(C.c_int32)), w.ctypes.data_as(C.POINTER(C.c_float)), C.c_int32(sl),
                                         lens.ctypes.data_as(C.POINTER(C.c_int32)), info.ctypes.data_as(C.POINTER(C.c_uint8))))
        self._n_pairs, self._seq_len, self._lens = n, sl, lens
        return lens, info

    def columns(self, pair: int, side: int) -> np.ndarray:
        n = int(self._lens[pair, side])
        out = np.zeros((n, self.P + 2), dtype=np.float32)
        api._check(_lib().twl_level_read_columns(self._h, C.c_int32(pair), C.c_int32(side), out.ctypes.data_as(C.POINTER(C.c_float)), C.c_int32(n)))
        return out

    def align(self, params: api.TwlParams, run_mask: Optional[np.ndarray] = None, zero_gap: Optional[np.ndarray] = None):
        n, sl = self._n_pairs, self._seq_len
        aln = np.zeros((n, 2 * sl), dtype=np.int8)
        aln_len = np.zeros(n, dtype=np.int32)
        err = np.zeros(n, dtype=np.int16)
        mask = None
        if run_mask is not None:
            m = np.ascontiguousarray(run_mask, dtype=np.uint8)
            mask = m.ctypes.data_as(C.POINTER(C.c_uint8))
        if zero_gap is not None:
            z = np.ascontiguousarray(zero_gap, dtype=np.uint8)
            assert z.shape == (n,)
            api._check(_lib().twl_level_align_mixed(self._h, C.byref(params), mask, z.ctypes.data_as(C.POINTER(C.c_uint8)), aln.ctypes.data_as(C.POINTER(C.c_int8)),
                                                    aln_len.ctypes.data_as(C.POINTER(C.c_int32)), err.ctypes.data_as(C.POINTER(C.c_int16))))
            return aln, aln_len, err
        api._check(_lib().twl_level_align(self._h, C.byref(params), mask, aln.ctypes.data_as(C.POINTER(C.c_int8)),
                                          aln_len.ctypes.data_as(C.POINTER(C.c_int32)), err.ctypes.data_as(C.POINTER(C.c_int16))))
        return aln, aln_len, err

    def align_in_hbm(self, params: api.TwlParams, run_mask: Optional[np.ndarray] = None):
        n = self._n_pairs
        aln_len = np.zeros(n, dtype=np.int32)
        err = np.zeros(n, dtype=np.int16)
        mask = None
        if run_mask is not None:
            m = np.ascontiguousarray(run_mask, dtype=np.uint8)
            mask = m.ctypes.data_as(C.POINTER(C.c_uint8))
        api._check(_lib().twl_level_align(self._h, C.byref(params), mask, None, aln_len.ctypes.data_as(C.POINTER(C.c_int32)), err.ctypes.data_as(C.POINTER(C.c_int16))))
        return aln_len, err

    def read_path(self, pair: int, length: int) -> np.ndarray:
        out = np.zeros(max(1, length), dtype=np.int8)
        api._check(_lib().twl_level_read_path(self._h, C.c_int32(pair), out.ctypes.data_as(C.POINTER(C.c_int8)), C.c_int32(length)))
        return out[:length]

    def restore(self, params: api.TwlParams, pairs: Sequence[int], out_stride: int) -> np.ndarray:
        sel = np.asarray(list(pairs), dtype=np.int32)
        out = np.zeros(max(1, len(sel)), dtype=np.int32)
        api._check(_lib().twl_level_restore(self._h, C.byref(params), C.c_int32(len(sel)), sel.ctypes.data_as(C.POINTER(C.c_int32)), C.c_int32(out_stride),
                                            out.ctypes.data_as(C.POINTER(C.c_int32))))
        return out[: len(sel)]

    def read_final(self, pair: int, length: int) -> np.ndarray:
        out = np.zeros(max(1, length), dtype=np.int8)
        api._check(_lib().twl_level_read_final(self._h, C.c_int32(pair), out.ctypes.data_as(C.POINTER(C.c_int8)), C.c_int32(length)))
        return out[:length]

    def write_final(self, pair: int, path: np.ndarray):
        p = np.ascontiguousarray(path, dtype=np.int8)
        api._check(_lib().twl_level_write_final(self._h, C.c_int32(pair), p.ctypes.data_as(C.POINTER(C.c_int8)), C.c_int32(len(p))))

    def exchange_buffers(self, send_bytes: int, recv_bytes: int):
        send, recv = C.c_void_p(), C.c_void_p()
        api._check(_lib().twl_level_exchange_buffers(self._h, C.c_int64(send_bytes), C.c_int64(recv_bytes), C.byref(send), C.byref(recv)))
        return int(send.value or 0), int(recv.value or 0)

    @staticmethod
    def _row_tables(pairs, lens, offsets):
        if pairs is None:
            return None, None, None, ()
        keep = (np.asarray(list(pairs), dtype=np.int32), np.asarray(list(lens), dtype=np.int32), np.asarray(list(offsets), dtype=np.int64))
        assert len(keep[0]) == len(keep[1]) == len(keep[2])
        return keep[0].ctypes.data_as(C.POINTER(C.c_int32)), keep[1].ctypes.data_as(C.POINTER(C.c_int32)), keep[2].ctypes.data_as(C.POINTER(C.c_int64)), keep

    def paths_to_block(self, pairs, lens, where, blk_ptr: int, offsets, n_sel: Optional[int] = None):
        pp, lp, op, keep = self._row_tables(pairs, lens, offsets)
        w = None if where is None else np.asarray(list(where), dtype=np.uint8)
        n = len(keep[0]) if n_sel is None and keep else int(n_sel or 0)
        api._check(_lib().twl_level_paths_to_block(self._h, C.c_int32(n), pp, lp, None if w is None else w.ctypes.data_as(C.POINTER(C.c_uint8)), C.c_void_p(blk_ptr), op))

    def paths_from_block(self, pairs, lens, blk_ptr: int, offsets, n_sel: Optional[int] = None):
        pp, lp, op, keep = self._row_tables(pairs, lens, offsets)
        n = len(keep[0]) if n_sel is None and keep else int(n_sel or 0)
        api._check(_lib().twl_level_paths_from_block(self._h, C.c_int32(n), pp, lp, C.c_void_p(blk_ptr), op))

    def commit_from_dp(self, paths: Sequence[Optional[np.ndarray]], path_len: Sequence[int], stride: Optional[int] = None, restored: Sequence[int] = ()):
        n = self._n_pairs
        stride = int(stride) if stride else max([1] + [int(x) for x in path_len])
        flat = np.zeros((n, stride), dtype=np.int8)
        plen = np.asarray(path_len, dtype=np.int32).copy()
        from_dp = np.zeros(n, dtype=np.uint8)
        for i, p in enumerate(paths):
            if p is None: from_dp[i] = (2 if i in set(restored) else 1) if plen[i] > 0 else 0
            else: flat[i, : len(p)] = p
        api._check(_lib().twl_level_commit_from_dp(self._h, flat.ctypes.data_as(C.POINTER(C.c_int8)), plen.ctypes.data_as(C.POINTER(C.c_int32)), C.c_int32(stride),
                                                   from_dp.ctypes.data_as(C.POINTER(C.c_uint8))))

    def commit(self, paths: Sequence[np.ndarray]):
        n = self._n_pairs
        assert len(paths) == n
        stride = max([1] + [len(p) for p in paths])
        flat = np.zeros((n, stride), dtype=np.int8)
        plen = np.zeros(n, dtype=np.int32)
        for i, p in enumerate(paths):
            flat[i, : len(p)] = p
            plen[i] = len(p)
        api._check(_lib().twl_level_commit(self._h, flat.ctypes.data_as(C.POINTER(C.c_int8)), plen.ctypes.data_as(C.POINTER(C.c_int32)), C.c_int32(stride)))
```

Measured before the change: 239.5 billion.

## Enqueue profile restore kernels behind DP collect in a combined align+restore call

Adds twl_level_align_restore, which queues the restore kernels on the stream right after the alignment collect kernel, so the host waits on one synchronisation instead of two. The restore kernel now skips pairs whose alignment failed, using the device error array. Read-back also reuses the cached lengths and errors instead of copying them again. The queued path is behind a new knob that defaults to off, so by default the combined call falls back to align-then-restore, and the host still routes eligible levels through it.

```diff
diff --git a/__graft_entry__.py b/__graft_entry__.py
--- a/__graft_entry__.py
+++ b/__graft_entry__.py
@@ -8,7 +8,7 @@
 CSRC = os.path.join(ROOT, "twilight_amd", "csrc")
 LIB = os.path.join(ROOT, "twilight_amd", "libtwl_align.so")
 HIPCC = os.environ.get("HIPCC", "/opt/rocm/bin/hipcc")
-KERNEL_SOURCES = ("twl_align.hip", "twl_knobs.inc.hip", "twl_launch.inc.hip", "twl_policy.inc.hip", "twl_run.inc.hip", "twl_comm.inc.hip", "talco_exit.hip.h", "talco_kernel.hip.h", "talco_nuc.hip.h", "talco_lds.hip.h", "talco_div.hip.h", "talco_team.hip.h", "talco_mt.hip.h", "talco_global.hip.h", "twl_level_plan.inc.hip", "twl_store.inc.hip", "twl_level.inc.hip", "level_kernels.hip.h", "restore_kernels.hip.h", "twl_place.inc.hip", "place_kernels.hip.h",
+KERNEL_SOURCES = ("twl_align.hip", "twl_knobs.inc.hip", "twl_launch.inc.hip", "twl_policy.inc.hip", "twl_run.inc.hip", "twl_comm.inc.hip", "talco_exit.hip.h", "talco_kernel.hip.h", "talco_nuc.hip.h", "talco_lds.hip.h", "talco_div.hip.h", "talco_team.hip.h", "talco_mt.hip.h", "talco_global.hip.h", "twl_level_plan.inc.hip", "twl_level_defer_plan.inc.hip", "twl_store.inc.hip", "twl_level.inc.hip", "level_kernels.hip.h", "restore_kernels.hip.h", "twl_place.inc.hip", "place_kernels.hip.h",
                   "twl_merge.inc.hip", "twl_merge_plan.inc.hip", "merge_kernels.hip.h", "twl_path_source.inc.hip", "twl_place_plan.inc.hip",
                   "twl_subtree.inc.hip", "twl_subtree_plan.inc.hip", "subtree_kernels.hip.h",
                   "twl_guide.inc.hip", "twl_guide_plan.inc.hip", "guide_kernels.hip.h",
diff --git a/include/twl_align.h b/include/twl_align.h
--- a/include/twl_align.h
+++ b/include/twl_align.h
@@ -99,7 +99,7 @@
 
 enum twl_knob { TWL_KNOB_MT_PERTURB = 1, TWL_KNOB_MT_MAX_PAIRS = 2, TWL_KNOB_MT_MIN_MARKER = 3, TWL_KNOB_MT_LEAD = 4, TWL_KNOB_MT_MARGIN = 5,
                 TWL_KNOB_MT_ROUNDS = 6, TWL_KNOB_MT_THR_JOBS = 7, TWL_KNOB_FAIL_ROW_ALLOCS = 8,
-                TWL_KNOB_PROT_MODE = 9, TWL_KNOB_ASSUME_ONEHOT_QUERY = 10, TWL_KNOB_MT_TAIL_PCT = 11, TWL_KNOB_MT_WIDE = 12, TWL_KNOB_NO_SPEC = 13, TWL_KNOB_SCOUT_XDROP_PCT = 14, TWL_KNOB_THR_SMALL = 15, TWL_KNOB_FORCE_GLOBAL = 16, TWL_KNOB_LEAF_STEP = 17, TWL_KNOB_POISON_TB = 18, TWL_KNOB_MT_ANCHOR = 19, TWL_KNOB_MT_LEAD2 = 20, TWL_KNOB_PROT_CORRIDOR = 21, TWL_KNOB_TAIL_OVERLAP = 22 };
+                TWL_KNOB_PROT_MODE = 9, TWL_KNOB_ASSUME_ONEHOT_QUERY = 10, TWL_KNOB_MT_TAIL_PCT = 11, TWL_KNOB_MT_WIDE = 12, TWL_KNOB_NO_SPEC = 13, TWL_KNOB_SCOUT_XDROP_PCT = 14, TWL_KNOB_THR_SMALL = 15, TWL_KNOB_FORCE_GLOBAL = 16, TWL_KNOB_LEAF_STEP = 17, TWL_KNOB_POISON_TB = 18, TWL_KNOB_MT_ANCHOR = 19, TWL_KNOB_MT_LEAD2 = 20, TWL_KNOB_PROT_CORRIDOR = 21, TWL_KNOB_TAIL_OVERLAP = 22, TWL_KNOB_LEVEL_DEFER = 23 };
 int twl_set_knob(int key, int value);
 int twl_plan_describe(const twl_params *p, int32_t n_pairs, const int32_t *len, int32_t num_cu, int32_t qry_onehot, int32_t wide_streak, char *out, int32_t cap);
 
diff --git a/include/twl_level.h b/include/twl_level.h
--- a/include/twl_level.h
+++ b/include/twl_level.h
@@ -45,6 +45,9 @@
 int twl_level_read_paths(twl_store *s, int32_t n_sel, const int32_t *pairs, const int32_t *lens, int8_t *out, int32_t out_stride);
 
 int twl_level_restore(twl_store *s, const twl_params *p, int32_t n_sel, const int32_t *pairs, int32_t out_stride, int32_t *final_len_out);
+int twl_level_align_restore(twl_store *s, const twl_params *p, const uint8_t *run_mask, const uint8_t *zero_gap, int32_t n_sel, const int32_t *pairs, int32_t out_stride,
+                            int32_t *aln_len_out, int16_t *err_out, int32_t *final_len_out);
+int twl_level_defer_counts(twl_store *s, int64_t *queued_out, int64_t *fell_back_out);
 int twl_level_exchange_buffers(twl_store *s, int64_t send_bytes, int64_t recv_bytes, void **send_dev, void **recv_dev);
 int twl_level_paths_to_block(twl_store *s, int32_t n_sel, const int32_t *pairs, const int32_t *lens, const uint8_t *where, void *blk_dev, const int64_t *blk_off);
 int twl_level_paths_from_block(twl_store *s, int32_t n_sel, const int32_t *pairs, const int32_t *lens, const void *blk_dev, const int64_t *blk_off);
diff --git a/twilight_amd/api.py b/twilight_amd/api.py
--- a/twilight_amd/api.py
+++ b/twilight_amd/api.py
@@ -151,6 +151,7 @@
 KNOB_PROT_CORRIDOR = 21
 KNOB_MT_LEAD2 = 20
 KNOB_TAIL_OVERLAP = 22
+KNOB_LEVEL_DEFER = 23
 PROT_MODES = {"auto": 0, "dense": 1, "sparse": 2, "presim": 3, "r1": 4, "lean_sparse": 5, "lean_presim": 6}
 
 
diff --git a/twilight_amd/csrc/host/align_resident.cpp b/twilight_amd/csrc/host/align_resident.cpp
--- a/twilight_amd/csrc/host/align_resident.cpp
+++ b/twilight_amd/csrc/host/align_resident.cpp
@@ -9,6 +9,9 @@
 #include <iostream>
 #include <string>
 #include <thread>
+
+extern "C" __attribute__((weak)) int twl_level_align_restore(twl_store *s, const twl_params *p, const uint8_t *run_mask, const uint8_t *zero_gap, int32_t n_sel,
+                                                             const int32_t *pairs, int32_t out_stride, int32_t *aln_len_out, int16_t *err_out, int32_t *final_len_out);
 
 namespace msa {
 namespace progressive {
@@ -317,7 +320,7 @@
 }
 
 int sortResults(const Level &lv, int d, const std::vector<uint8_t> &mask, const int8_t *aln, const std::vector<int32_t> &alnLen, const std::vector<int16_t> &err,
-                PairRows &rows, ReplicaShare &mine)
+                PairRows &rows, ReplicaShare &mine, const std::vector<int32_t> *cand = nullptr, const std::vector<int32_t> *candFin = nullptr)
 {
     const size_t pitch = (size_t)2 * lv.stride;
     std::vector<int32_t> restore, restoreLen;
@@ -333,8 +336,16 @@
     }
     if (restore.empty()) return (int)TWL_OK;
     std::vector<int32_t> fin(restore.size(), -1);
-    const int rc = twl_level_restore(lv.ctx.stores[d], &lv.tp, (int32_t)restore.size(), restore.data(), lv.pathStride, fin.data());
-    if (rc != TWL_OK) return rc;
+    if (cand) {
+        for (size_t t = 0, c = 0; t < restore.size(); ++t, ++c) {
+            while (c < cand->size() && (*cand)[c] != restore[t]) ++c;
+            if (c == cand->size()) { std::cerr << "ERROR: a pair to restore was not given to twl_level_align_restore.\n"; exit(1); }
+            fin[t] = (*candFin)[c];
+        }
+    } else {
+        const int rc = twl_level_restore(lv.ctx.stores[d], &lv.tp, (int32_t)restore.size(), restore.data(), lv.pathStride, fin.data());
+        if (rc != TWL_OK) return rc;
+    }
     for (size_t t = 0; t < restore.size(); ++t) {
         if (fin[t] > 0) { rows.fromDp[restore[t]] = 2; rows.dpLen[restore[t]] = fin[t]; }
         else { mine.handedBack.push_back(restore[t]); mine.handedBackLen.push_back(restoreLen[t]); }
@@ -352,9 +363,16 @@
     int8_t *aln = lv.route.inPlace ? nullptr : reinterpret_cast<int8_t *>(g_alnStage[d].get((size_t)n * 2 * lv.stride));
     std::vector<int32_t> alnLen(n);
     std::vector<int16_t> err(n);
+    std::vector<int32_t> cand, candFin;
+    if (lv.route.inPlace && !lv.route.procs && lv.task == 0 && twl_level_align_restore != nullptr)
+        for (int i = 0; i < n; ++i)
+            if (mask[i] && lv.needsHost[i] && !deferredLowQuality(lv.task, lv.ps[i])) cand.push_back(i);
+    candFin.assign(cand.size(), 0);
+    const twl_params *prm = (cntZero == cnt) ? &lv.tz : &lv.tp;
+    const uint8_t *zero = (cntZero == cnt || !cntZero) ? nullptr : lv.maskZero.data();
     const double tCall = nowMs();
-    const int rc = (cntZero == cnt) ? twl_level_align(lv.ctx.stores[d], &lv.tz, mask.data(), aln, alnLen.data(), err.data())
-                                    : twl_level_align_mixed(lv.ctx.stores[d], &lv.tp, mask.data(), cntZero ? lv.maskZero.data() : nullptr, aln, alnLen.data(), err.data());
+    const int rc = !cand.empty() ? twl_level_align_restore(lv.ctx.stores[d], prm, mask.data(), zero, (int32_t)cand.size(), cand.data(), lv.pathStride, alnLen.data(), err.data(), candFin.data())
+                                 : twl_level_align_mixed(lv.ctx.stores[d], prm, mask.data(), zero, aln, alnLen.data(), err.data());
     if (rc != TWL_OK) return rc;
     mine.callMs += nowMs() - tCall;
     addStats(lv, d, true, mine);
@@ -362,7 +380,7 @@
         const int rr = retryDeferredPair(lv, d, mask, aln, alnLen, err, mine);
         if (rr != TWL_OK) return rr;
     }
-    return sortResults(lv, d, mask, aln, alnLen, err, rows, mine);
+    return cand.empty() ? sortResults(lv, d, mask, aln, alnLen, err, rows, mine) : sortResults(lv, d, mask, aln, alnLen, err, rows, mine, &cand, &candFin);
 }
 
 #ifdef TWL_DEV
diff --git a/twilight_amd/csrc/restore_kernels.hip.h b/twilight_amd/csrc/restore_kernels.hip.h
--- a/twilight_amd/csrc/restore_kernels.hip.h
+++ b/twilight_amd/csrc/restore_kernels.hip.h
@@ -9,6 +9,7 @@
 struct RestoreArgs {
     const int8_t *aln;
     const int32_t *aln_len;
+    const int16_t *err;
     int32_t aln_stride;
     const uint8_t *colinfo;
     int32_t stride;
@@ -69,6 +70,10 @@
     __shared__ int s_big;
     const int pair = a.sel[blockIdx.x];
     const int n = a.aln_len[pair];
+    if (a.err && (a.err[pair] != 0 || n <= 0 || n > a.aln_stride)) {
+        if (threadIdx.x == 0) { a.out_len[pair] = -1; a.n_both[blockIdx.x] = 0; }
+        return;
+    }
     const int8_t *path = a.aln + (size_t)pair * a.aln_stride;
     const int32_t *oiR = a.orig_idx + (size_t)(2 * blockIdx.x) * (size_t)(a.stride + 1), *oiQ = oiR + (a.stride + 1);
     int32_t *runR = a.run + (size_t)blockIdx.x * 4 * a.bstride, *runQ = runR + a.bstride, *stR = runQ + a.bstride, *stQ = stR + a.bstride;
diff --git a/twilight_amd/csrc/twl_align.hip b/twilight_amd/csrc/twl_align.hip
--- a/twilight_amd/csrc/twl_align.hip
+++ b/twilight_amd/csrc/twl_align.hip
@@ -103,6 +103,8 @@
     }
     void release() { if (p) (void)hipFree(p); p = nullptr; cap = 0; }
 };
+
+struct BehindCollect { int (*fn)(void *ctx, hipStream_t st) = nullptr; void *ctx = nullptr; bool ran = false; };
 
 struct Device {
     int id = 0;
@@ -145,6 +147,7 @@
     twl::FillArgs fills{};
     char *res_h = nullptr; size_t res_cap = 0;
     std::vector<int32_t> last_alnlen;
+    BehindCollect *behind_collect = nullptr;
     std::mutex mu;
 };
 
@@ -359,9 +362,12 @@
     if (rc) return rc;
     std::vector<int32_t> alen((size_t)n);
     std::vector<int16_t> aerr((size_t)n);
-    HIP_TRY(hipMemcpyAsync(alen.data(), d->d_alnlen.p, alen.size() * sizeof(int32_t), hipMemcpyDeviceToHost, st));
-    HIP_TRY(hipMemcpyAsync(aerr.data(), d->d_err.p, aerr.size() * sizeof(int16_t), hipMemcpyDeviceToHost, st));
-    HIP_TRY(hipStreamSynchronize(st));
+    if ((int32_t)d->last_err.size() == n && (int32_t)d->last_alnlen.size() == n) { alen = d->last_alnlen; aerr = d->last_err; }
+    else {
+        HIP_TRY(hipMemcpyAsync(alen.data(), d->d_alnlen.p, alen.size() * sizeof(int32_t), hipMemcpyDeviceToHost, st));
+        HIP_TRY(hipMemcpyAsync(aerr.data(), d->d_err.p, aerr.size() * sizeof(int16_t), hipMemcpyDeviceToHost, st));
+        HIP_TRY(hipStreamSynchronize(st));
+    }
     size_t path_bytes = 0;
     for (int32_t t = 0; t < n; ++t) path_bytes += (size_t)std::max(alen[t], 0);
     const bool bulk = contiguous && path_bytes * 8 >= (size_t)n * 2 * sl;
@@ -594,6 +600,7 @@
     case TWL_KNOB_PROT_CORRIDOR: g_prot_corridor = std::max(0, value); for (auto *d : g_devs) d->mem.forget_corridor(); return TWL_OK;
     case TWL_KNOB_SCOUT_XDROP_PCT: g_scout_xdrop_pct = std::max(10, std::min(100, value)); return TWL_OK;
     case TWL_KNOB_TAIL_OVERLAP: g_tail_overlap = value ? 1 : 0; return TWL_OK;
+    case TWL_KNOB_LEVEL_DEFER: g_level_defer = value ? 1 : 0; return TWL_OK;
     case TWL_KNOB_THR_SMALL: g_thr_small = std::max(0, std::min(2, value)); for (auto *d : g_devs) d->mem.forget_small(); return TWL_OK;
     default: g_err = "unknown knob"; return TWL_ERR_BAD_ARGUMENT;
     }
@@ -652,6 +659,7 @@
 }
 
 #include "twl_level_plan.inc.hip"
+#include "twl_level_defer_plan.inc.hip"
 #include "twl_store.inc.hip"
 #include "twl_level.inc.hip"
 #include "twl_place.inc.hip"
diff --git a/twilight_amd/csrc/twl_knobs.inc.hip b/twilight_amd/csrc/twl_knobs.inc.hip
--- a/twilight_amd/csrc/twl_knobs.inc.hip
+++ b/twilight_amd/csrc/twl_knobs.inc.hip
@@ -16,6 +16,7 @@
 int g_leaf_step = 1;
 int g_poison_tb = 0;
 int g_tail_overlap = 1;
+int g_level_defer = 0;
 Knobs current_knobs()
 {
     return Knobs{g_mt_max_pairs, g_mt_min_marker, g_mt_tail_pct, g_mt_wide, g_assume_onehot_query, g_no_spec, g_thr_small, (ProtMode)g_prot_mode, g_prot_corridor,
diff --git a/twilight_amd/csrc/twl_level.inc.hip b/twilight_amd/csrc/twl_level.inc.hip
--- a/twilight_amd/csrc/twl_level.inc.hip
+++ b/twilight_amd/csrc/twl_level.inc.hip
@@ -191,39 +191,71 @@
     return a;
 }
 
-int restore_batch(twl_store *s, const twl_params *p, int32_t n_sel, const int32_t *pairs, int32_t out_stride, int32_t *final_len_out)
+struct RestoreLaunch {
+    twl::RestoreArgs a{};
+    unsigned nWch = 0, nb = 0;
+    bool handedBack = false;
+    twl_store *s = nullptr;
+};
+
+int restore_setup(twl_store *s, const twl_params *p, int32_t n_sel, const int32_t *pairs, int32_t out_stride, const int16_t *errs, RestoreLaunch &rl)
 {
     int rc;
     const int32_t n = s->n_pairs;
     hipStream_t st = s->d->stream;
     LevelBufs *lv = s->lv;
     const size_t bstride = 2 * (size_t)s->seq_len + 1;
+    rl.s = s;
     {
         Arena &A = lv->up_restore;
         if ((rc = A.begin((size_t)n_sel * sizeof(int32_t), 1))) return rc;
         A.put(lv->r_sel, pairs, (size_t)n_sel);
         if ((rc = A.flush(st))) return rc;
     }
-    const unsigned nWch = (unsigned)((bstride + (size_t)twl::kRsThreads * twl::kWrItems - 1) / ((size_t)twl::kRsThreads * twl::kWrItems));
-    const unsigned nb = (unsigned)std::max(1, std::min(128, 4096 / n_sel));
+    rl.nWch = (unsigned)((bstride + (size_t)twl::kRsThreads * twl::kWrItems - 1) / ((size_t)twl::kRsThreads * twl::kWrItems));
+    rl.nb = (unsigned)std::max(1, std::min(128, 4096 / n_sel));
     bool soft = false;
-    if ((rc = size_restore(lv, (size_t)n_sel, (size_t)n, (size_t)s->seq_len, nWch, nb, soft))) {
+    if ((rc = size_restore(lv, (size_t)n_sel, (size_t)n, (size_t)s->seq_len, rl.nWch, rl.nb, soft))) {
         if (!soft) return rc;
         (void)hipGetLastError();
+        rl.handedBack = true;
+        return TWL_OK;
+    }
+    if ((rc = lv->back.ensure((size_t)n * sizeof(int32_t)))) return rc;
+    rl.a = restore_args(s, p, n_sel, out_stride, rl.nWch);
+    rl.a.err = errs;
+    return TWL_OK;
+}
+
+int restore_enqueue(const RestoreLaunch &rl, hipStream_t st)
+{
+    const twl::RestoreArgs &a = rl.a;
+    const unsigned n_sel = (unsigned)a.n_sel;
+    LevelBufs *lv = rl.s->lv;
+    hipLaunchKernelGGL(twl::restore_index_kernel, dim3(2 * n_sel), dim3(twl::kRsThreads), 0, st, a);
+    hipLaunchKernelGGL(twl::restore_runs_kernel, dim3(n_sel), dim3(twl::kRsThreads), 0, st, a);
+    hipLaunchKernelGGL(twl::restore_align_kernel, dim3(n_sel, rl.nb), dim3(twl::kNwThreads), 0, st, a);
+    hipLaunchKernelGGL(twl::restore_count_kernel, dim3(n_sel, rl.nWch), dim3(twl::kRsThreads), 0, st, a);
+    hipLaunchKernelGGL(twl::restore_write_kernel, dim3(n_sel, rl.nWch), dim3(twl::kRsThreads), 0, st, a);
+    HIP_TRY(hipGetLastError());
+    HIP_TRY(hipMemcpyAsync(lv->back.p, lv->r_outlen.p, (size_t)rl.s->n_pairs * sizeof(int32_t), hipMemcpyDeviceToHost, st));
+    return TWL_OK;
+}
+int restore_enqueue_hook(void *ctx, hipStream_t st) { return restore_enqueue(*static_cast<const RestoreLaunch *>(ctx), st); }
+
+int restore_batch(twl_store *s, const twl_params *p, int32_t n_sel, const int32_t *pairs, int32_t out_stride, int32_t *final_len_out)
+{
+    int rc;
+    hipStream_t st = s->d->stream;
+    RestoreLaunch rl;
+    if ((rc = restore_setup(s, p, n_sel, pairs, out_stride, nullptr, rl))) return rc;
+    if (rl.handedBack) {
         for (int32_t t = 0; t < n_sel; ++t) final_len_out[t] = -1;
         return TWL_OK;
     }
-    const twl::RestoreArgs a = restore_args(s, p, n_sel, out_stride, nWch);
-    hipLaunchKernelGGL(twl::restore_index_kernel, dim3(2 * (unsigned)n_sel), dim3(twl::kRsThreads), 0, st, a);
-    hipLaunchKernelGGL(twl::restore_runs_kernel, dim3((unsigned)n_sel), dim3(twl::kRsThreads), 0, st, a);
-    hipLaunchKernelGGL(twl::restore_align_kernel, dim3((unsigned)n_sel, nb), dim3(twl::kNwThreads), 0, st, a);
-    hipLaunchKernelGGL(twl::restore_count_kernel, dim3((unsigned)n_sel, nWch), dim3(twl::kRsThreads), 0, st, a);
-    hipLaunchKernelGGL(twl::restore_write_kernel, dim3((unsigned)n_sel, nWch), dim3(twl::kRsThreads), 0, st, a);
-    HIP_TRY(hipGetLastError());
-    if ((rc = lv->back.ensure((size_t)n * sizeof(int32_t)))) return rc;
-    HIP_TRY(hipMemcpyAsync(lv->back.p, lv->r_outlen.p, (size_t)n * sizeof(int32_t), hipMemcpyDeviceToHost, st));
+    if ((rc = restore_enqueue(rl, st))) return rc;
     HIP_TRY(hipStreamSynchronize(st));
-    const int32_t *all = (const int32_t *)lv->back.p;
+    const int32_t *all = (const int32_t *)s->lv->back.p;
     for (int32_t t = 0; t < n_sel; ++t) final_len_out[t] = all[pairs[t]];
     return TWL_OK;
 }
@@ -507,9 +539,79 @@
     if (s->staged_stride && s->staged_stride != out_stride) { g_err = "twl_level_restore: one row pitch per level"; return TWL_ERR_BAD_ARGUMENT; }
     if ((rc = s->lv->d_paths.ensure((size_t)n * (size_t)out_stride))) return rc;
     s->staged_stride = out_stride;
-    constexpr int32_t kBatch = 4096;
+    constexpr int32_t kBatch = defer::kRestoreBatch;
     for (int32_t at = 0; at < n_sel; at += kBatch)
         if ((rc = restore_batch(s, p, std::min(kBatch, n_sel - at), pairs + at, out_stride, final_len_out + at))) return rc;
+    return TWL_OK;
+}
+
+namespace {
+int align_restore_queued(twl_store *s, const twl_params *p, const uint8_t *run_mask, const uint8_t *zero_gap, int32_t n_sel, const int32_t *pairs, int32_t out_stride,
+                         int32_t *aln_len_out, int16_t *err_out, int32_t *final_len_out, bool *dpDone, bool *stands)
+{
+    const int32_t n = s->n_pairs;
+    DEVICE_CALL(call, s->d);
+    Device *d = call.d;
+    hipStream_t st = call.st;
+    LevelBufs *lv = s->lv;
+    int rc;
+    if ((rc = lv->d_paths.ensure((size_t)n * (size_t)out_stride))) return rc;
+    s->staged_stride = out_stride;
+    const AlignPlan ap = plan_align(n, s->h_len, s->sides.data(), run_mask, g_leaf_step);
+    if ((rc = upload_align(lv, st, ap.lm))) return rc;
+    if ((rc = size_align(lv, (size_t)n, (size_t)s->seq_len))) return rc;
+    RestoreLaunch rl;
+    if ((rc = restore_setup(s, p, n_sel, pairs, out_stride, (const int16_t *)lv->d_err.p, rl))) return rc;
+    if (rl.handedBack) return TWL_OK;
+    BehindCollect hook;
+    hook.fn = restore_enqueue_hook; hook.ctx = &rl;
+    HIP_TRY(hipEventRecord(d->ev[5], st));
+    d->behind_collect = &hook;
+    rc = run_device(d, st, p, n, s->seq_len, nullptr, nullptr, nullptr, lv->d_lenmask.as<const int32_t>(), lv->d_num.as<const int32_t>(), (int8_t *)lv->d_aln.p,
+                    (int32_t *)lv->d_alnlen.p, (int16_t *)lv->d_err.p, ap.lm.data(), (const float *)lv->d_cols.p, ap.qryOneHot, zero_gap, ap.shape);
+    d->behind_collect = nullptr;
+    if (rc) return rc;
+    if ((rc = read_back_align(s, d, st, nullptr, aln_len_out, err_out))) return rc;
+    *dpDone = true;
+    *stands = defer::restore_stands(true, hook.ran, d->stats.n_launches);
+    if (!*stands) return TWL_OK;
+    const int32_t *all = (const int32_t *)lv->back.p;
+    for (int32_t t = 0; t < n_sel; ++t) final_len_out[t] = defer::final_len(err_out[pairs[t]], aln_len_out[pairs[t]], all[pairs[t]]);
+    return TWL_OK;
+}
+}
+
+int twl_level_align_restore(twl_store *s, const twl_params *p, const uint8_t *run_mask, const uint8_t *zero_gap, int32_t n_sel, const int32_t *pairs, int32_t out_stride,
+                            int32_t *aln_len_out, int16_t *err_out, int32_t *final_len_out)
+{
+    if (!s || !s->prepared) { g_err = "twl_level_prepare has not been called"; return TWL_ERR_BAD_ARGUMENT; }
+    int rc = check_params(p);
+    if (rc) return rc;
+    if (p->P != s->P) { g_err = "params.P does not match the store's sequence type"; return TWL_ERR_BAD_ARGUMENT; }
+    const int32_t n = s->n_pairs;
+    if (n_sel < 0 || (n_sel > 0 && (!pairs || !final_len_out)) || out_stride < 1 || (n > 0 && (!aln_len_out || !err_out))) { g_err = "bad argument"; return TWL_ERR_BAD_ARGUMENT; }
+    for (int32_t t = 0; t < n_sel; ++t) if (pairs[t] < 0 || pairs[t] >= n) { g_err = "pair index out of range"; return TWL_ERR_BAD_ARGUMENT; }
+    if (s->staged_stride && s->staged_stride != out_stride) { g_err = "twl_level_restore: one row pitch per level"; return TWL_ERR_BAD_ARGUMENT; }
+    if (n == 0) return TWL_OK;
+    bool dpDone = false, stands = false;
+    const bool queued = defer::queue_restore(g_level_defer, n_sel, n);
+    if (queued && (rc = align_restore_queued(s, p, run_mask, zero_gap, n_sel, pairs, out_stride, aln_len_out, err_out, final_len_out, &dpDone, &stands))) return rc;
+    if (stands) { ++s->defer_taken; return TWL_OK; }
+    if (queued) ++s->defer_fell_back;
+    if (!dpDone && (rc = twl_level_align_mixed(s, p, run_mask, zero_gap, nullptr, aln_len_out, err_out))) return rc;
+    std::vector<int32_t> sel((size_t)n_sel), slot((size_t)n_sel), fin((size_t)n_sel, -1);
+    const int32_t m = defer::restorable(n_sel, pairs, err_out, aln_len_out, sel.data(), slot.data());
+    if ((rc = twl_level_restore(s, p, m, sel.data(), out_stride, fin.data()))) return rc;
+    for (int32_t t = 0; t < n_sel; ++t) final_len_out[t] = 0;
+    for (int32_t k = 0; k < m; ++k) final_len_out[slot[k]] = defer::final_len(0, aln_len_out[sel[k]], fin[k]);
+    return TWL_OK;
+}
+
+int twl_level_defer_counts(twl_store *s, int64_t *queued_out, int64_t *fell_back_out)
+{
+    if (!s) { g_err = "store is null"; return TWL_ERR_BAD_ARGUMENT; }
+    if (queued_out) *queued_out = s->defer_taken;
+    if (fell_back_out) *fell_back_out = s->defer_fell_back;
     return TWL_OK;
 }
 
diff --git a/twilight_amd/csrc/twl_level_defer_plan.inc.hip b/twilight_amd/csrc/twl_level_defer_plan.inc.hip
--- /dev/null
+++ b/twilight_amd/csrc/twl_level_defer_plan.inc.hip
@@ -0,0 +1,32 @@
+#pragma once
+#include <cstdint>
+
+namespace defer {
+
+constexpr int32_t kRestoreBatch = 4096;
+
+inline bool queue_restore(int knob, int32_t n_sel, int32_t n_pairs)
+{
+    return knob != 0 && n_sel > 0 && n_sel <= kRestoreBatch && n_sel <= n_pairs;
+}
+
+inline bool restore_stands(bool queued, bool launched, int32_t n_launches)
+{
+    return queued && launched && n_launches == 1;
+}
+
+inline int32_t final_len(int16_t err, int32_t aln_len, int32_t out_len)
+{
+    if (err != 0 || aln_len <= 0) return 0;
+    return out_len > 0 ? out_len : -1;
+}
+
+inline int32_t restorable(int32_t n_sel, const int32_t *pairs, const int16_t *err, const int32_t *aln_len, int32_t *out_pairs, int32_t *slot)
+{
+    int32_t m = 0;
+    for (int32_t t = 0; t < n_sel; ++t)
+        if (err[pairs[t]] == 0 && aln_len[pairs[t]] > 0) { out_pairs[m] = pairs[t]; slot[m] = t; ++m; }
+    return m;
+}
+
+}
diff --git a/twilight_amd/csrc/twl_run.inc.hip b/twilight_amd/csrc/twl_run.inc.hip
--- a/twilight_amd/csrc/twl_run.inc.hip
+++ b/twilight_amd/csrc/twl_run.inc.hip
@@ -271,6 +271,11 @@
     hipLaunchKernelGGL(twl::collect_kernel, dim3((unsigned)((n_pairs + 255) / 256)), dim3(256), 0, c.st, (int)n_pairs, (const int16_t *)c.d_err, (const int32_t *)c.d_alnlen,
                        (const unsigned long long *)d->cells.p, withMt ? (const unsigned long long *)d->mt_stat.p : nullptr, (unsigned long long *)d->res_h);
     HIP_TRY(hipGetLastError());
+    if (BehindCollect *h = d->behind_collect) {
+        d->behind_collect = nullptr;
+        h->ran = true;
+        if (const int rc = h->fn(h->ctx, c.st)) return rc;
+    }
     HIP_TRY(hipStreamSynchronize(c.st));
     const unsigned long long *r = (const unsigned long long *)d->res_h;
     const int32_t *rl = (const int32_t *)(r + 4 + n_pairs);
diff --git a/twilight_amd/csrc/twl_store.inc.hip b/twilight_amd/csrc/twl_store.inc.hip
--- a/twilight_amd/csrc/twl_store.inc.hip
+++ b/twilight_amd/csrc/twl_store.inc.hip
@@ -207,6 +207,7 @@
     hipEvent_t rows_event = nullptr;
     LevelBufs *lv = nullptr;
     int32_t staged_stride = 0;
+    int64_t defer_taken = 0, defer_fell_back = 0;
     Arena up_rows;
     Buf d_gather;
     Buf x_send, x_recv;
diff --git a/twilight_amd/level.py b/twilight_amd/level.py
--- a/twilight_amd/level.py
+++ b/twilight_amd/level.py
@@ -17,7 +17,7 @@
 _SYMBOLS = ["twl_store_create", "twl_store_destroy", "twl_store_read_rows", "twl_store_read_rows_of", "twl_store_write_rows", "twl_store_write_cache", "twl_store_rows_to_block", "twl_store_rows_from_block", "twl_store_exchange_buffers", "twl_store_read_cache", "twl_store_drop_cache",
             "twl_level_prepare", "twl_level_read_colinfo", "twl_level_read_colinfo_many", "twl_level_align", "twl_level_align_mixed", "twl_level_read_path", "twl_level_read_paths", "twl_level_commit", "twl_level_commit_from_dp", "twl_level_read_columns", "twl_level_timing",
             "twl_level_restore", "twl_level_read_final", "twl_level_exchange_buffers", "twl_level_paths_to_block", "twl_level_paths_from_block",
-            "twl_level_write_final"]
+            "twl_level_write_final", "twl_level_align_restore", "twl_level_defer_counts"]
 
 
 def exported_symbols():
@@ -210,6 +210,25 @@
                                             out.ctypes.data_as(C.POINTER(C.c_int32))))
         return out[: len(sel)]
 
+    def align_restore(self, params: api.TwlParams, pairs: Sequence[int], out_stride: int, run_mask: Optional[np.ndarray] = None, zero_gap: Optional[np.ndarray] = None):
+        n = self._n_pairs
+        aln_len = np.zeros(n, dtype=np.int32)
+        err = np.zeros(n, dtype=np.int16)
+        sel = np.asarray(list(pairs), dtype=np.int32)
+        fin = np.zeros(max(1, len(sel)), dtype=np.int32)
+        m = None if run_mask is None else np.ascontiguousarray(run_mask, dtype=np.uint8)
+        z = None if zero_gap is None else np.ascontiguousarray(zero_gap, dtype=np.uint8)
+        api._check(_lib().twl_level_align_restore(self._h, C.byref(params), None if m is None else m.ctypes.data_as(C.POINTER(C.c_uint8)),
+                                                  None if z is None else z.ctypes.data_as(C.POINTER(C.c_uint8)), C.c_int32(len(sel)), sel.ctypes.data_as(C.POINTER(C.c_int32)),
+                                                  C.c_int32(out_stride), aln_len.ctypes.data_as(C.POINTER(C.c_int32)), err.ctypes.data_as(C.POINTER(C.c_int16)),
+                                                  fin.ctypes.data_as(C.POINTER(C.c_int32))))
+        return aln_len, err, fin[: len(sel)]
+
+    def defer_counts(self):
+        a, b = C.c_int64(0), C.c_int64(0)
+        api._check(_lib().twl_level_defer_counts(self._h, C.byref(a), C.byref(b)))
+        return int(a.value), int(b.value)
+
     def read_final(self, pair: int, length: int) -> np.ndarray:
         out = np.zeros(max(1, length), dtype=np.int8)
         api._check(_lib().twl_level_read_final(self._h, C.c_int32(pair), out.ctypes.data_as(C.POINTER(C.c_int8)), C.c_int32(length)))
```

Result: no change. 239.3 billion (-0.1%).
